# vxlerian/cpu-raymarcher

Hardware: AMD Instinct MI355X
Metric: frames/sec, 3840x2160 Dense-Grid sphere-trace (+ avg SDF-calls/pixel) (higher is better)
Workload: dtype f64

## Files before the change

### cpu_raymarcher_amd/_native.py

```python
import ctypes as C
import os
import subprocess

_PKG = os.path.dirname(os.path.abspath(__file__))
LIB_PATH = os.environ.get("RM_HIP_LIB") or os.path.join(_PKG, "librm_hip.so")
CSRC = os.path.join(_PKG, "csrc")

RM_OK = 0
RM_E_INVALID = -1
RM_E_UNSUPPORTED = -2
RM_E_NO_DEVICE = -3
RM_E_HIP = -4
RM_E_NO_SCENE = -5
RM_E_NOMEM = -6
RM_SCENE_UPLOADED = -(2 ** 31)

_STATUS_NAMES = {0: "RM_OK", -1: "RM_E_INVALID", -2: "RM_E_UNSUPPORTED", -3: "RM_E_NO_DEVICE",
                 -4: "RM_E_HIP", -5: "RM_E_NO_SCENE", -6: "RM_E_NOMEM"}


class RmError(RuntimeError):
    def __init__(self, code, msg):
        super().__init__("%s (%d): %s" % (_STATUS_NAMES.get(code, "?"), code, msg))
        self.code = code
# ... 207 lines not shown
    "rm_scene_field_device": (C.c_int, [_VP, C.POINTER(rm_lattice), _VP, _VP, _VP, _VP]),
    "rm_scene_points": (C.c_int, [_VP, C.POINTER(rm_point_query), C.c_int64, _VP, _VP, _VP, _VP, _VP, _VP, _VP]),
    "rm_scene_points_device": (C.c_int, [_VP, C.POINTER(rm_point_query), C.c_int64, _VP, _VP, _VP, _VP, _VP, _VP, _VP, _VP]),
    "rm_lattice_points": (C.c_int, [C.POINTER(rm_lattice), C.c_int64, C.c_int64, _VP]),
    "rm_shade_field_device": (C.c_int, [_VP, C.POINTER(rm_field_shade), C.c_int64, _VP, _VP, _VP]),
    "rm_shade_field": (C.c_int, [_VP, C.POINTER(rm_field_shade), C.c_int64, _VP, _VP]),
    "rm_mesh_field_device": (C.c_int, [_VP, C.POINTER(rm_lattice), _VP, C.c_int32, C.c_double, _VP, C.c_int64, _VP, C.c_int64, _VP, _VP]),
    "rm_scene_mesh": (C.c_int, [_VP, C.POINTER(rm_lattice), C.c_double, _VP, C.c_int64, _VP, C.c_int64, C.POINTER(rm_mesh_info)]),
    "rm_mesh_cells_device": (C.c_int, [_VP, C.POINTER(rm_lattice), _VP, C.c_int32, C.c_double, _VP, C.c_int64, _VP, _VP]),
    "rm_scene_sharpen_device": (C.c_int, [_VP, C.POINTER(rm_lattice), C.POINTER(rm_sharp_query), C.c_int64, _VP, _VP, _VP, _VP, _VP]),
    "rm_scene_sharpen": (C.c_int, [_VP, C.POINTER(rm_lattice), C.POINTER(rm_sharp_query), C.c_int64, _VP, _VP, _VP, _VP]),
    "rm_lattice_blocks": (C.c_int, [C.POINTER(rm_lattice), C.POINTER(C.c_int32)]),
    "rm_scene_blocks_device": (C.c_int, [_VP, C.POINTER(rm_lattice), C.c_double, C.c_double, _VP, _VP, _VP, _VP, _VP]),
    "rm_scene_tiles_device": (C.c_int, [_VP, C.POINTER(rm_lattice), _VP, C.c_int64, _VP, _VP]),
    "rm_scene_edit_balls": (C.c_int, [_VP, C.POINTER(rm_sphere_edit), C.c_int32, C.POINTER(rm_ball), C.c_int32, C.POINTER(C.c_int32)]),
    "rm_scene_tiles_update_device": (C.c_int, [_VP, C.POINTER(rm_lattice), _VP, _VP, C.c_int64, _VP, C.c_int32, _VP, C.c_int64, _VP, _VP, _VP, _VP]),
    "rm_mesh_tiles_device": (C.c_int, [_VP, C.POINTER(rm_lattice), _VP, _VP, C.c_int64, _VP, C.c_double, _VP, C.c_int64, _VP, C.c_int64, _VP, _VP,
                                       _VP, _VP]),
    "rm_scene_mesh_sparse": (C.c_int, [_VP, C.POINTER(rm_lattice), C.c_double, C.c_double, _VP, C.c_int64, _VP, C.c_int64, _VP, _VP,
                                       C.POINTER(rm_mesh_info), C.POINTER(rm_sparse_info)]),
    "rm_measure_field_device": (C.c_int, [_VP, C.POINTER(rm_lattice), _VP, C.c_int32, C.c_double, _VP, _VP]),
    "rm_measure_tiles_device": (C.c_int, [_VP, C.POINTER(rm_lattice), _VP, _VP, C.c_int64, _VP, _VP, C.c_double, _VP, _VP]),
    "rm_scene_measure": (C.c_int, [_VP, C.POINTER(rm_lattice), C.c_double, C.c_double, C.POINTER(rm_measure), C.POINTER(rm_sparse_info)]),
    "rm_measure_world": (C.c_int, [C.POINTER(rm_lattice), C.POINTER(rm_measure), C.POINTER(rm_measure_world)]),
    "rm_label_field_device": (C.c_int, [_VP, C.POINTER(rm_lattice), _VP, C.c_int32, C.c_double, C.c_int32, _VP, _VP, _VP]),
    "rm_measure_labels_device": (C.c_int, [_VP, C.POINTER(rm_lattice), _VP, C.c_int64, _VP, _VP]),
    "rm_scene_parts": (C.c_int, [_VP, C.POINTER(rm_lattice), C.c_double, C.c_int32, _VP, C.c_int64, _VP, C.POINTER(rm_parts_info)]),
    "rm_ray_march": (C.c_int, [_VP, C.POINTER(rm_ray_query), C.c_int64, _VP, _VP, _VP, _VP, _VP, _VP]),
    "rm_ray_march_device": (C.c_int, [_VP, C.POINTER(rm_ray_query), C.c_int64, _VP, _VP, _VP, _VP, _VP, _VP, _VP]),
    "rm_camera_rays": (C.c_int, [C.c_int32, C.c_int32, C.c_double, C.c_double, C.c_int32, C.c_int32, _VP, _VP]),
    "rm_ray_pick": (C.c_int, [_VP, C.POINTER(rm_ray_query), C.c_int64, _VP, _VP, _VP, _VP, _VP, _VP, _VP]),
    "rm_ray_pick_device": (C.c_int, [_VP, C.POINTER(rm_ray_query), C.c_int64, _VP, _VP, _VP, _VP, _VP, _VP, _VP, _VP]),
    "rm_ray_light": (C.c_int, [_VP, C.POINTER(rm_ray_query), C.POINTER(rm_light), C.c_int64, _VP, _VP, _VP, _VP, _VP, _VP, _VP, _VP, _VP,
                               _VP]),
    "rm_ray_light_device": (C.c_int, [_VP, C.POINTER(rm_ray_query), C.POINTER(rm_light), C.c_int64, _VP, _VP, _VP, _VP, _VP, _VP, _VP, _VP,
                                      _VP, _VP, _VP]),
    "rm_ray_walk": (C.c_int, [_VP, C.POINTER(rm_ray_query), C.c_int64, _VP, _VP, C.c_int32, _VP, _VP]),
    "rm_ray_walk_device": (C.c_int, [_VP, C.POINTER(rm_ray_query), C.c_int64, _VP, _VP, C.c_int32, _VP, _VP, _VP]),
    "rm_phong_light": (C.c_int, [_VP]),
    "rm_shade_lit_device": (C.c_int, [_VP, C.c_int32, C.c_int32, C.c_int32, _VP, _VP, _VP, _VP, _VP, _VP]),
    "rm_shade_lit": (C.c_int, [_VP, C.c_int32, C.c_int32, C.c_int32, _VP, _VP, _VP, _VP, _VP]),
    "rm_scene_object": (C.c_int, [_VP, C.c_int32, C.POINTER(rm_node), C.c_int32, C.POINTER(C.c_int32)]),
    "rm_render_tile": (C.c_int, [_VP, C.POINTER(rm_job), _VP, _VP, _VP, _VP]),
    "rm_render_tile_device": (C.c_int, [_VP, C.POINTER(rm_job), C.c_int32, _VP, _VP, _VP, _VP, _VP, _VP]),
    "rm_render_frames_device": (C.c_int, [_VP, C.POINTER(rm_job), C.c_int32, _VP, C.c_int32, _VP, _VP, _VP, _VP, _VP, _VP, _VP]),
    "rm_compare_frames_device": (C.c_int, [_VP, C.c_int32, C.c_int32, C.c_int32, C.POINTER(rm_frame_set), C.POINTER(rm_frame_set),
                                           C.c_int32, C.c_int32, _VP, _VP, _VP]),
    "rm_compare_frames": (C.c_int, [_VP, C.c_int32, C.c_int32, C.c_int32, C.POINTER(rm_frame_set), C.POINTER(rm_frame_set),
                                    C.c_int32, C.c_int32, _VP, _VP]),
    "rm_counter_hist_device": (C.c_int, [_VP, C.c_int32, C.c_int32, C.c_int32, _VP, _VP, _VP, C.c_int32, C.c_int32, C.c_int32, C.c_int32,
                                         _VP, _VP]),
    "rm_counter_hist": (C.c_int, [_VP, C.c_int32, C.c_int32, C.c_int32, _VP, _VP, _VP, C.c_int32, C.c_int32, C.c_int32, C.c_int32, _VP]),
    "rm_shade_ranged_device": (C.c_int, [_VP, C.c_int32, C.c_int32, C.c_int32, C.c_int32, _VP, _VP, C.c_uint32, C.c_uint32, _VP, _VP]),
    "rm_shade_ranged": (C.c_int, [_VP, C.c_int32, C.c_int32, C.c_int32, C.c_int32, _VP, _VP, C.c_uint32, C.c_uint32, _VP]),
    "rm_sweep_views": (C.c_int, [C.c_double, C.c_double, C.c_double, C.c_double, C.c_double, C.c_double, C.c_int32, _VP]),
    "rm_render_stripes_device": (C.c_int, [_VP, C.POINTER(rm_job), C.c_int32, C.c_int32, C.c_int32, C.c_int32,
                                           _VP, _VP, _VP, _VP, _VP, _VP]),
    "rm_stripe_rows": (C.c_int, [C.c_int32, C.c_int32, C.c_int32, C.c_int32, C.c_int32]),
    "rm_deal_stripes": (C.c_int, [C.c_int32, C.c_int32, C.c_int32, _VP, _VP]),
    "rm_render_stripe_list_device": (C.c_int, [_VP, C.POINTER(rm_job), C.c_int32, C.c_int32, _VP, C.c_int32,
                                               _VP, _VP, _VP, _VP, _VP, _VP]),
    "rm_assemble_frame_device": (C.c_int, [_VP, _VP, C.c_int64, C.c_int64, C.c_int32, C.c_int32, C.c_int32, _VP,
                                           C.c_int32, C.c_int32, _VP, C.c_int64, _VP, _VP]),
    "rm_shade": (C.c_int, [_VP, C.c_int32, C.c_int32, C.c_int32, _VP, _VP, _VP, _VP, _VP]),
    "rm_shade_device": (C.c_int, [_VP, C.c_int32, C.c_int32, C.c_int32, _VP, _VP, _VP, _VP, _VP, _VP]),
    "rm_reduce_counters": (C.c_int, [_VP, _VP, _VP, C.c_int64, C.POINTER(rm_diagnostics)]),
    "rm_reduce_counters_device": (C.c_int, [_VP, _VP, _VP, C.c_int64, C.POINTER(rm_diagnostics), _VP]),
    "rm_reduce_counters_enqueue": (C.c_int, [_VP, _VP, _VP, C.c_int64, _VP, _VP]),
    "rm_render_attach_diagnostics": (C.c_int, [_VP, _VP]),
    "rm_partition_rows": (C.c_int, [C.c_int32, C.c_int32, C.c_int32, C.POINTER(C.c_int32), C.POINTER(C.c_int32)]),
    "rm_selftest_hypot": (C.c_int, [_VP, _VP, C.c_int64, _VP]),
    "rm_selftest_fastdiv": (C.c_int, [_VP, C.c_uint64, C.c_int64, C.POINTER(C.c_uint64)]),
    "rm_selftest_recip": (C.c_int, [_VP, C.c_int, _VP]),
    "rm_debug_read_stamps": (C.c_int, [_VP, _VP]),
    "rm_debug_read_wave_times": (C.c_int, [_VP, _VP]),
    "rm_debug_read_batch_log": (C.c_int, [_VP, _VP]),
    "rm_debug_read_counts": (C.c_int, [_VP, _VP]),
    "rm_debug_read_lpt_costs": (C.c_int, [_VP, _VP, C.c_int64]),
    "rm_debug_launch_fill": (C.c_int, [_VP, C.c_int32, C.POINTER(C.c_int32)]),
    "rm_debug_last_launch": (C.c_int, [_VP, C.POINTER(C.c_uint32)]),
    "rm_debug_overlap_fill": (C.c_int, [_VP, C.c_int32, C.c_int64, C.POINTER(C.c_int32)]),
    "rm_debug_step_box": (C.c_int, [_VP, C.POINTER(C.c_int32)]),
    "rm_debug_cell_tab": (C.c_int, [_VP, C.POINTER(C.c_int32)]),
    "rm_debug_exact_tree": (C.c_int, [_VP, C.POINTER(C.c_int32)]),
    "rm_debug_rect_cull": (C.c_int, [_VP, _VP, _VP, C.c_int32, C.c_int32, C.POINTER(C.c_int32)]),
    "rm_debug_leaf_rects": (C.c_int, [_VP, _VP, _VP, C.c_int32, C.c_int32, _VP, _VP, C.c_int64, C.POINTER(C.c_int64)]),
    "rm_rtc_source": (C.c_int, [_VP, C.c_char_p, C.c_int64, C.POINTER(C.c_int64)]),
    "rm_rtc_compile_check": (C.c_int, [_VP, C.c_int32, C.c_int32, C.c_char_p, C.c_int64, C.POINTER(C.c_double)]),
    "rm_rtc_status": (C.c_int, [_VP, C.POINTER(C.c_int32), C.POINTER(C.c_int32), C.c_char_p, C.c_int64]),
    "rm_set_option": (C.c_int, [_VP, C.c_char_p, C.c_int64]),
    "rm_get_option": (C.c_int, [_VP, C.c_char_p, C.POINTER(C.c_int64)]),
}

_lib = None


def build(force=False, verbose=False):
    srcs = [os.path.join(CSRC, f) for f in os.listdir(CSRC) if f.endswith((".hip", ".cpp", ".h"))]
    srcs.append(os.path.join(os.path.dirname(_PKG), "include", "rm_raymarch.h"))
    if not force and os.path.exists(LIB_PATH) and all(
            os.path.getmtime(LIB_PATH) >= os.path.getmtime(s) for s in srcs):
        return LIB_PATH
    cmd = ["make", "-j%d" % min(8, os.cpu_count() or 1), "-C", CSRC, "all"] + (["-B"] if force else [])
    subprocess.check_call(cmd, stdout=None if verbose else subprocess.DEVNULL)
    return LIB_PATH


def lib():
    global _lib
    if _lib is None:
        if not os.path.exists(LIB_PATH):
            raise ImportError(
                "cpu_raymarcher_amd: %s is missing. Build it with `python -c 'import __graft_entry__ as g; "
                "g.build()'` or `make -C cpu_raymarcher_amd/csrc`. There is no CPU fallback." % LIB_PATH)
        try:
            import torch
        except ImportError:
            pass
        L = C.CDLL(LIB_PATH)
        for name, (res, args) in SIGNATURES.items():
            if os.environ.get("RM_HIP_LIB") and not hasattr(L, name):
                continue
            fn = getattr(L, name)
            fn.restype = res
            fn.argtypes = args
        _lib = L
    return _lib


def check(ctx, rc):
    if rc == RM_OK:
        return
    msg = lib().rm_last_error(ctx).decode() if ctx else ""
    raise (RmUnsupported if rc == RM_E_UNSUPPORTED else RmError)(rc, msg)
```

### cpu_raymarcher_amd/context.py

```python
import collections
import contextlib
import ctypes as C

import numpy as np

from . import _native as N

Points = collections.namedtuple("Points", "position dist normal object steps count")
SparseBlocks = collections.namedtuple("SparseBlocks", "slot list dist n_kept dims")
Sharp = collections.namedtuple("Sharp", "position feature count")
MeasureWorld = collections.namedtuple("MeasureWorld", "cell_volume volume centroid second projected_area area_estimate")


class Measure(collections.namedtuple("Measure", "n_points n_inside n_nonfinite sum1 sum2 crossings lo hi n_blocks n_kept n_blocks_inside")):
    world = None

    def inertia(self):
        xx, yy, zz, xy, yz, zx = self.world.second
        second = np.array([[xx, xy, zx], [xy, yy, yz], [zx, yz, zz]], np.float64)
        return np.trace(second) * np.eye(3) - second


class Parts:

# ... 128 lines not shown


def _current_stream_ptr():
    import torch
    return C.c_void_p(torch.cuda.current_stream().cuda_stream)


class Context:

    def __init__(self, device=0):
        self._h = C.c_void_p()
        self.device = -1 if device is None else int(device)
        rc = N.lib().rm_create(self.device, C.byref(self._h))
        if rc != N.RM_OK:
            raise N.RmError(rc, "rm_create(device=%d) failed: no usable HIP device" % self.device)

    def close(self):
        if self._h:
            N.lib().rm_destroy(self._h)
            self._h = C.c_void_p()

    def __del__(self):
        try:
            self.close()
        except Exception:
            pass

    def __enter__(self):
        return self

    def __exit__(self, *a):
        self.close()

    def set_option(self, key, value):
        N.check(self._h, N.lib().rm_set_option(self._h, key.encode(), int(value)))

    def get_option(self, key):
        v = C.c_int64(0)
        N.check(self._h, N.lib().rm_get_option(self._h, key.encode(), C.byref(v)))
        return v.value

    @contextlib.contextmanager
    def _exact(self, exact):
        if not exact:
            yield
            return
        before = self.get_option("exact")
        self.set_option("exact", 1)
        try:
            yield
        finally:
            self.set_option("exact", before)

    def exact_tree(self):
        out = (C.c_int32 * 4)()
        N.check(self._h, N.lib().rm_debug_exact_tree(self._h, out))
        return dict(mode=out[0], nodes=out[1], leaves=out[2], depth=out[3])

    def launch_fill(self, asked):
        v = C.c_int32(0)
        N.check(self._h, N.lib().rm_debug_launch_fill(self._h, int(asked), C.byref(v)))
        return v.value

    def last_launch(self):
        out = (C.c_uint32 * 4)()
        N.check(self._h, N.lib().rm_debug_last_launch(self._h, out))
        return dict(workgroups=out[0], threads=out[1], lds_bytes=out[2], cus=out[3])

    def overlap_fill(self, asked, items):
        v = C.c_int32(0)
        N.check(self._h, N.lib().rm_debug_overlap_fill(self._h, int(asked), int(items), C.byref(v)))
        return v.value

    def step_box(self):
        out = (C.c_int32 * 6)()
        N.check(self._h, N.lib().rm_debug_step_box(self._h, out))
        return dict(last=bool(out[0]), planned=bool(out[1]), reason=out[2], list_cap=out[3], list_cap_without=out[4], table_bytes=out[5])

    def cell_tab(self):
        out = (C.c_int32 * 12)()
        N.check(self._h, N.lib().rm_debug_cell_tab(self._h, out))
        return dict(last=bool(out[0]), planned=bool(out[1]), reason=out[2], list_cap=out[3], list_cap_without=out[4], table_bytes=out[5],
                    per_cu=out[6], scene_bytes=out[7], scene_bytes_without=out[8], cells=out[9], records=out[10], leaf_sets=out[11])

    def rect_cull(self, rot, origin, width, height):
        r = np.ascontiguousarray(rot, dtype=np.float32).reshape(9)
        o = np.ascontiguousarray(origin, dtype=np.float32).reshape(3)
        out = (C.c_int32 * 5)()
        N.check(self._h, N.lib().rm_debug_rect_cull(self._h, _ptr(r), _ptr(o), int(width), int(height), out))
        return dict(last=bool(out[0]), planned=bool(out[1]), reason=out[2], leaves=out[3], max_leaves=out[4])

    def leaf_rects(self, rot, origin, width, height):
        r = np.ascontiguousarray(rot, dtype=np.float32).reshape(9)
        o = np.ascontiguousarray(origin, dtype=np.float32).reshape(3)
        n = C.c_int64(0)
        N.check(self._h, N.lib().rm_debug_leaf_rects(self._h, _ptr(r), _ptr(o), int(width), int(height), None, None, 0, C.byref(n)))
        rects = np.zeros((max(1, n.value), 4), np.uint16)
        nodes = np.zeros(max(1, n.value), np.int32)
        N.check(self._h, N.lib().rm_debug_leaf_rects(self._h, _ptr(r), _ptr(o), int(width), int(height), _ptr(rects), _ptr(nodes),
                                                     n.value, C.byref(n)))
        return rects[:n.value], nodes[:n.value]

    def scene_from_preset(self, index, accel):
        N.check(self._h, N.lib().rm_scene_from_preset(self._h, int(index), int(accel)))

    def scene_from_spheres(self, centers, radii, accel):
        c = np.ascontiguousarray(centers, dtype=np.float32).reshape(-1, 3)
        r = np.ascontiguousarray(radii, dtype=np.float64).reshape(-1)
        if len(c) != len(r):
            raise ValueError("centers and radii differ in length")
        N.check(self._h, N.lib().rm_scene_from_spheres(self._h, _ptr(c), _ptr(r), len(r), int(accel)))

    def scene_from_prims(self, prims, accel):
        prims = list(prims)
        arr = (N.rm_prim * max(1, len(prims)))()
        for i, (t, m, par) in enumerate(prims):
            arr[i].type = int(t)
            for k in range(16):
                arr[i].world_to_local[k] = float(m[k])
            for k in range(3):
                arr[i].params[k] = float(par[k]) if k < len(par) else 0.0
        N.check(self._h, N.lib().rm_scene_from_prims(self._h, arr, len(prims), int(accel)))

    def scene_from_nodes(self, nodes, roots, accel):
        nodes = list(nodes)
        arr = (N.rm_node * max(1, len(nodes)))()
        for i, (t, a, b, m, par) in enumerate(nodes):
            arr[i].type, arr[i].child_a, arr[i].child_b = int(t), int(a), int(b)
            for k in range(16):
                arr[i].world_to_local[k] = 0.0 if m is None else float(m[k])
            for k in range(6):
                arr[i].params[k] = float(par[k]) if k < len(par) else 0.0
        r = np.ascontiguousarray(roots, dtype=np.int32)
        N.check(self._h, N.lib().rm_scene_from_nodes(self._h, arr, len(nodes), _ptr(r), len(r), int(accel)))

    def edit_spheres(self, edits):
        arr, n = self._edit_array(edits)
        N.check(self._h, N.lib().rm_scene_edit_spheres(self._h, arr, n))

    @staticmethod
    def _edit_array(edits):
        if isinstance(edits, C.Array) and edits._type_ is N.rm_sphere_edit:
            return edits, len(edits)
        edits = list(edits)
        n = len(edits)
        arr = (N.rm_sphere_edit * max(1, n))()
        for k, e in enumerate(edits):
            arr[k].op = N.EDIT_OPS[e[0]] if isinstance(e[0], str) else int(e[0])
            arr[k].index = int(e[1])
            if len(e) > 2:
                arr[k].center[:] = [float(v) for v in np.asarray(e[2], np.float32).reshape(3)]
                arr[k].radius = float(e[3])
        return arr, n

    def edit_balls(self, edits):
        arr, n = self._edit_array(edits)
        count = C.c_int32(0)
        out = np.zeros(2 * n, N.BALL_DTYPE)
        N.check(self._h, N.lib().rm_scene_edit_balls(self._h, arr, n, out.ctypes.data_as(C.POINTER(N.rm_ball)) if n else None, 2 * n, C.byref(count)))
        return out[:count.value]

    def scene_table(self, name, from_device=True):
        size = C.c_int64(0)
        key = name.encode()
        N.check(self._h, N.lib().rm_debug_scene_table(self._h, key, int(bool(from_device)), None, 0, C.byref(size)))
        out = np.zeros(size.value, np.uint8)
# ... 1126 lines not shown
```

### cpu_raymarcher_amd/csrc/rm_api.cpp

```cpp
#include <hip/hip_runtime_api.h>

#include <algorithm>
#include <array>
#include <cerrno>
#include <climits>
#include <cmath>
#include <cstdio>
#include <cstdlib>
#include <cstring>
#include <functional>
#include <limits>
#include <map>
#include <unordered_map>
#include <new>
#include <string>
#include <vector>

#include "../../include/rm_raymarch.h"
#include "rm_diag.h"
#include "rm_kernels.h"
#include "rm_rtc.h"
#include "rm_scene_host.h"

namespace {
// ... 260 lines not shown
        for (auto &u : t.users) {
            (void)hipEventSynchronize(u.second);
            (void)hipEventDestroy(u.second);
        }
        t.users.clear();
        t.valid = false;
        const size_t n = static_cast<size_t>(oct_nodes);
        if (t.nodes < n) {
            (void)hipFree(t.dev);
            t.dev = nullptr;
            t.nodes = 0;
            if (hipMalloc(reinterpret_cast<void **>(&t.dev), n * sizeof(RmOctFrameNode)) == hipSuccess) t.nodes = n;
            else (void)hipGetLastError();
        }
        if (!t.dev || rm_launch_oct_frame_table(oct, oct_nodes, origin, t.dev, stream) != hipSuccess) return nullptr;
        for (int a = 0; a < 3; ++a) t.origin[a] = origin[a];
        t.gen = gen;
        t.valid = true;
        t.builder = stream;
        if (!t.built && hipEventCreateWithFlags(&t.built, hipEventDisableTiming) != hipSuccess) t.built = nullptr;
        if (!t.built || hipEventRecord(t.built, stream) != hipSuccess) (void)hipStreamSynchronize(stream);
        cur = k;
        return &t;
    }
    static void read_by(Table &t, hipStream_t stream) {
        hipEvent_t ev = nullptr;
        for (auto &u : t.users)
            if (u.first == stream) ev = u.second;
        if (!ev) {
            if (hipEventCreateWithFlags(&ev, hipEventDisableTiming) == hipSuccess) t.users.emplace_back(stream, ev);
            else ev = nullptr;
        }
        if (ev) (void)hipEventRecord(ev, stream);
        else (void)hipStreamSynchronize(stream);
    }
    void release() {
        for (Table &t : slots) {
            (void)hipFree(t.dev);
            for (auto &u : t.users) (void)hipEventDestroy(u.second);
            if (t.built) (void)hipEventDestroy(t.built);
        }
    }
};

}

struct rm_ctx {
    int device = -1;
    bool has_device = false;
    std::string err = "";
    hipStream_t stream = nullptr;

    bool have_scene = false;
    bool scene_is_uploaded = false;
    int scene_preset = 0;
    rmh::HostScene host;
    DeviceScene dev;

    bool have_uploaded = false;
    SceneDesc uploaded;
    double time = 0.0;

    void *scratch = nullptr;
    size_t scratch_bytes = 0;
    hipEvent_t scratch_busy = nullptr;
    RmDiagDevice *d_diag = nullptr;
    float light[3] = {0, 0, 0};

    int64_t opt_tile_w = 8;
    bool tile_w_set = false;
    int64_t opt_filter = 1;
    int64_t opt_lds = 1;
    int64_t opt_kernel = 0;
    int64_t opt_list_cap = 32;
    int64_t opt_coop = 1;
    int64_t opt_grid = 1;
    int64_t opt_nn = 2;
    int64_t opt_ext = 1;
    int64_t opt_blocks_per_cu = 6;
    int64_t opt_lds_fill = 0;
    int64_t opt_min_fill = 1;
    int64_t opt_overlap_fill = 1;
    int hw_queues = 4;
    uint32_t last_v2_shape[6] = {0, 0, 0, 0, 0, 0};
    int64_t opt_item_wide = 0;
    int64_t opt_multi_step = 1;
    int64_t opt_step_box = 1;
    int64_t opt_cell_tab = 1;
    int64_t opt_lds_kb = 0;
    int64_t opt_refill = 64;
    int64_t opt_recs = 1;
    int64_t opt_static = 0;
    int64_t opt_lut = 1;
    int64_t opt_cull = 1;
    int64_t opt_rect_cull = 1;
    std::vector<uint16_t> cull_leaves;
    int64_t opt_rel = 1;
    int64_t opt_uniform = 1;
    int64_t opt_sub = 1;
    int64_t opt_hw_xcd = 1;
    int64_t opt_v1_lists = 1;
    int64_t opt_v1_block = 64;
    int64_t opt_oct_lean = 1;
    int64_t opt_lpt = 1;
    LaunchSlots slots;
    LptRing lpt;
    OctTableRing oct_tables;
    FrameRing frames;
    CompareRing compare;
    HistRing hists;
    unsigned long long scene_gen = 0;
    int64_t opt_n0_batch = 64;
    int64_t opt_length = 0;
    int64_t opt_exact = 0;
    bool exact_ready = false;
    int exact_mode = 0;
    rmh::ExactTree exact_tree;
    RmBvhNode *d_exact_nodes = nullptr;
    int32_t *d_exact_ids = nullptr;
    const char *last_kernel = "";
    std::string last_kernel_kept;
    int64_t opt_device_build = 1;
    int64_t opt_specialise = 1;
    int64_t opt_rtc_spheres = 16;
    int64_t opt_prune = 1;
    std::string rtc_src;
    std::map<int, rmrtc::Kernel> rtc_kernels;
    std::vector<rmrtc::Kernel> rtc_owned;
    std::map<int, std::string> rtc_failed;
    std::string rtc_log;
    struct V2Special {
        int launches = 0;
        int state = 0;
        bool lite = false;
        rmrtc::Kernel k;
    };
    std::unordered_map<uint64_t, V2Special> v2_special;
    int64_t opt_v2_after = 3;
    struct DevTable {
        std::vector<int32_t> host;
        int32_t *dev = nullptr;
    };
    std::vector<DevTable> tables;
    int64_t opt_item_px = 128;
    void *diag_next = nullptr;
    unsigned long long *d_stamps = nullptr;
    int num_cus = 256;
};

namespace {

int fail(rm_ctx *ctx, int code, const std::string &msg) {
    if (ctx) ctx->err = msg;
    return code;
}

int hip_fail(rm_ctx *ctx, hipError_t e, const char *what) {
    return fail(ctx, RM_E_HIP, std::string(what) + ": " + hipGetErrorString(e));
}

int read_hw_queues() {
    const char *s = std::getenv("GPU_MAX_HW_QUEUES");
    if (!s || !*s) return 4;
    char *end = nullptr;
    errno = 0;
    const long long v = std::strtoll(s, &end, 10);
    if (errno || end == s || *end != '\0' || v <= 0) return 4;
    return static_cast<int>(std::min<long long>(v, INT_MAX));
}

int launch_fill(int asked, int queues, bool min_fill) {
// ... 686 lines not shown
    std::memcpy(p.light, ctx->light, sizeof p.light);
    for (int k = 0; k < 9; ++k) p.rot_d[k] = p.rot[k];
    for (int k = 0; k < 3; ++k) {
        p.origin_d[k] = p.origin[k];
        p.light_d[k] = p.light[k];
    }
    fill_scene_view(ctx, p);
    if (!std::isfinite(job->time)) return fail(ctx, RM_E_INVALID, "non-finite time");
    ctx->time = job->time;
    p.time = job->time;
    p.tile_w = static_cast<int32_t>(ctx->opt_tile_w);
    p.nodes_in_lds = static_cast<int32_t>(ctx->opt_lds);
    p.filter = static_cast<int32_t>(ctx->opt_filter);
    p.variant = static_cast<int32_t>(ctx->opt_kernel);
    if (p.variant == 0)
        p.variant = (ctx->host.accel == RM_ACCEL_OCTREE || ctx->host.spheres.size() < 8 ||
                     (ctx->opt_specialise && !ctx->rtc_src.empty() && rmrtc::available(nullptr) &&
                      static_cast<int64_t>(ctx->host.spheres.size()) < ctx->opt_rtc_spheres))
                        ? 1
                        : 2;
    if (p.algorithm != RM_ALG_SPHERE_TRACER) p.variant = 1;
    if (ctx->host.general) p.variant = 1;
    if (p.variant == 1 && !ctx->tile_w_set) p.tile_w = 8;
    p.list_cap = static_cast<int32_t>(ctx->opt_list_cap);
    p.coop = static_cast<int32_t>(ctx->opt_coop);
    p.bvh_prim_count = static_cast<int32_t>(ctx->host.bvh_prims.size());
    p.oct_prim_count = static_cast<int32_t>(ctx->host.oct_prims.size());
    p.blocks_per_cu = static_cast<int32_t>(ctx->opt_blocks_per_cu);
    p.launch_per_cu = launch_fill(p.blocks_per_cu, ctx->hw_queues, ctx->opt_min_fill != 0);
    p.overlap_per_cu = overlap_fill(p.blocks_per_cu, ctx->hw_queues, ctx->opt_min_fill != 0, ctx->opt_overlap_fill != 0);
    p.num_cus = ctx->num_cus;
    p.refill_threshold = static_cast<int32_t>(ctx->opt_refill);
    p.hw_xcd = static_cast<int32_t>(ctx->opt_hw_xcd);
    p.item_px = static_cast<int32_t>(ctx->opt_item_px);
    p.stamps = ctx->d_stamps;
    for (int k = 0; k < 3; ++k) {
        p.pq_dim[k] = ctx->host.pq_dim[k];
        p.pq_origin[k] = ctx->host.pq_origin[k];
        p.pq_inv[k] = ctx->host.pq_inv[k];
        p.pq_cell[k] = ctx->host.pq_inv[k] > 0.f ? static_cast<float>((1.0 / static_cast<double>(ctx->host.pq_inv[k])) * 0.9999) : 0.f;
    }
    p.pq_cell_count = static_cast<int32_t>(ctx->host.pq_cells.size());
    p.pq_list_count = static_cast<int32_t>(ctx->host.pq_list.size());
    p.use_grid = (ctx->opt_grid && !ctx->host.pq_cells.empty()) ? 1 : 0;
    p.pq_cells = ctx->dev.pq_cells;
    p.pq_list = ctx->dev.pq_list;
    p.bvh_leaves = ctx->dev.bvh_leaves;
    p.bvh_leaf_count = (ctx->opt_cull && ctx->host.accel == RM_ACCEL_BVH) ? ctx->dev.bvh_leaf_count : 0;
    p.rect_cull = rect_cull_refusal(ctx, p.rot, p.origin, p.width, p.height) == 0 ? 1 : 0;
    p.nn_cells = ctx->dev.nn_cells;
    p.nn_list = ctx->dev.nn_list;
    p.nn_cell_count = static_cast<int32_t>(ctx->host.nn_cells.size());
    p.nn_list_count = static_cast<int32_t>(ctx->host.nn_list.size());
    const bool nn_on = ctx->opt_nn == 1 || (ctx->opt_nn == 2 && ctx->host.spheres.size() <= 512);
    p.use_nn = (p.use_grid && nn_on && !ctx->host.nn_cells.empty()) ? 1 : 0;
    p.leaf_order = ctx->host.leaf_order ? 1 : 0;
    p.rel_boxes = static_cast<int32_t>(ctx->opt_rel);
    p.n0_batch = static_cast<int32_t>(ctx->opt_n0_batch);
    p.v1_lists = static_cast<int32_t>(ctx->opt_v1_lists);
    p.v1_block = static_cast<int32_t>(ctx->opt_v1_block);
    p.oct_lean = static_cast<int32_t>(ctx->opt_oct_lean);
    p.v1_list_offset = -1;
    p.prim_filter = (ctx->opt_filter && ctx->host.general && !ctx->host.program && ctx->host.prim_filter_ok &&
                     ctx->host.spheres.size() == ctx->host.prims.size()) ? 1 : 0;
    p.lds_budget_kb = static_cast<int32_t>(ctx->opt_lds_kb);
    p.lds_fill = static_cast<int32_t>(ctx->opt_lds_fill);
    p.item_wide = static_cast<int32_t>(ctx->opt_item_wide);
    p.multi_step = static_cast<int32_t>(ctx->opt_multi_step);
    p.step_tab = ctx->dev.step_tab;
    p.sb_bins = ctx->host.sb_bins;
    p.sb_stride = ctx->host.sb_stride;
    for (int k = 0; k < 3; ++k) {
        p.sb_origin[k] = ctx->host.sb_origin[k];
        p.sb_inv[k] = ctx->host.sb_inv[k];
    }
    p.step_box = (ctx->opt_step_box && ctx->opt_multi_step && ctx->host.accel == RM_ACCEL_BVH && !ctx->host.step_tab.empty() &&
                  (ctx->dev.step_tab || !ctx->has_device)) ? 1 : 0;
    p.cell_tab = ctx->dev.cell_tab;
    p.ct_rec_off = ctx->host.ct_rec_off;
    p.ct_list_off = ctx->host.ct_list_off;
    p.ct_words = static_cast<int32_t>(ctx->host.cell_tab.size());
    for (int k = 0; k < 3; ++k) p.ct_dim[k] = ctx->host.ct_dim[k];
    p.cell_on = (ctx->opt_cell_tab && p.step_box && !ctx->host.cell_tab.empty() && (ctx->dev.cell_tab || !ctx->has_device)) ? 1 : 0;
    p.uniform_radius = 0;
    if (ctx->opt_uniform && !ctx->host.general && ctx->host.spheres.size() >= 2 &&
        ctx->host.spheres.size() <= 256) {
        const auto &sp = ctx->host.spheres;
        const auto &rd = ctx->host.radii;
        bool same = rd.size() == sp.size();
        for (size_t k = 1; same && k < sp.size(); ++k)
            same = std::memcmp(&sp[k].rf, &sp[0].rf, sizeof(float)) == 0 && std::memcmp(&rd[k], &rd[0], sizeof(double)) == 0;
        p.uniform_radius = same ? 1 : 0;
    }
    for (int k = 0; k < 3; ++k) {
        p.nn_dim[k] = ctx->host.nn_dim[k];
        p.nn_inv[k] = ctx->host.nn_inv[k];
    }
    p.oct_recs = ctx->opt_recs ? ctx->dev.oct_recs : nullptr;
    p.oct_sub_hdr = (ctx->opt_sub && ctx->opt_recs) ? ctx->dev.oct_sub_hdr : nullptr;
    p.oct_sub_list = ctx->dev.oct_sub_list;
    return RM_OK;
}

template <typename Launch>
int read_mismatches(rm_ctx *ctx, Launch launch, uint64_t *mismatches) {
    RM_HIP(ctx, hipSetDevice(ctx->device));
    Staging st{ctx};
    const size_t o = st.region(sizeof(unsigned long long));
    const int rc = st.reserve();
    if (rc) return rc;
    RM_HIP(ctx, st.zero(o, sizeof(unsigned long long)));
    RM_HIP(ctx, launch(st.at<unsigned long long>(o)));
    unsigned long long h = 0;
    RM_HIP(ctx, st.out(&h, o, sizeof h));
    RM_HIP(ctx, st.sync());
    *mismatches = h;
    return RM_OK;
}

int norm_shader(int s) { return (s >= RM_SHADE_NORMAL && s <= RM_SHADE_ITERATION_HEATMAP) ? s : RM_SHADE_NORMAL; }

int fill_query_params(rm_ctx *ctx, const rm_ray_query *q, RmRenderParams &p) {
    const double scene_time = ctx->time;
    rm_job job;
    std::memset(&job, 0, sizeof job);
    job.width = 1;
    job.height = 1;
    job.y_end = 1;
    job.time = q->time;
    const bool known = q->algorithm >= RM_ALG_SPHERE_TRACER && q->algorithm <= RM_ALG_ADAPTIVE_STEP_V3;
    job.algorithm = known ? q->algorithm : RM_ALG_SPHERE_TRACER;
    job.scene_preset_index = ctx->scene_is_uploaded ? RM_SCENE_UPLOADED : ctx->scene_preset;
    job.acceleration_structure = ctx->host.accel;
    job.overshoot_factor = q->overshoot_factor;
    job.step_size = q->step_size;
    const int rc = fill_params(ctx, &job, p);
    ctx->time = scene_time;
    p.rtc_function = nullptr;
    return rc;
}

int check_query(rm_ctx *ctx, const rm_ray_query *q, int64_t n, const void *origins, const void *dirs) {
    if (!q) return fail(ctx, RM_E_INVALID, "null query");
    if (n < 0 || n > std::numeric_limits<int32_t>::max()) return fail(ctx, RM_E_INVALID, "ray count out of range");
    if (n > 0 && (!origins || !dirs)) return fail(ctx, RM_E_INVALID, "null ray buffer");
    if (!ctx->has_device) return fail(ctx, RM_E_NO_DEVICE, "host-only context: there is no CPU ray path");
    if (!ctx->have_scene) return fail(ctx, RM_E_NO_SCENE, "no scene set");
    return RM_OK;
}

template <typename Args>
struct RayCall {
    RmRays rays;
    Args args;
    hipError_t (*launch[2])(const RmRenderParams &, const RmRays &, const Args &, hipStream_t, const char **);
    int64_t chunk;
    int n_cols;
    Column cols[kMaxColumns];
    void column(const void *ptr, size_t bytes, void *slot, bool in, bool out = true) { cols[n_cols++] = Column{ptr, bytes, slot, in, out}; }
};

template <typename Args, typename Check, typename Describe>
int ray_call(rm_ctx *ctx, const rm_ray_query *q, int64_t n, const void *origins, const void *dirs, bool host, void *stream, Check check,
             Describe describe) {
    if (!ctx) return RM_E_INVALID;
    int rc = check();
// ... 2405 lines not shown
    if (asked < 1 || asked > 8) return fail(ctx, RM_E_INVALID, "blocks_per_cu must be in [1, 8]");
    if (items < 0) return fail(ctx, RM_E_INVALID, "items must not be negative");
    const bool min_fill = ctx->opt_min_fill != 0;
    *effective = rm_v2_overlap_per_cu(launch_fill(asked, ctx->hw_queues, min_fill),
                                      overlap_fill(asked, ctx->hw_queues, min_fill, ctx->opt_overlap_fill != 0), items, ctx->num_cus);
    return RM_OK;
}

int rm_debug_last_launch(rm_ctx *ctx, uint32_t out[4]) {
    if (!ctx || !out) return RM_E_INVALID;
    for (int k = 0; k < 3; ++k) out[k] = ctx->last_v2_shape[k];
    out[3] = static_cast<uint32_t>(ctx->num_cus);
    return RM_OK;
}

int rm_debug_step_box(rm_ctx *ctx, int32_t out[6]) {
    if (!ctx || !out) return RM_E_INVALID;
    for (int k = 0; k < 6; ++k) out[k] = 0;
    out[0] = static_cast<int32_t>(ctx->last_v2_shape[3]);
    if (!ctx->have_scene) return fail(ctx, RM_E_NO_SCENE, "no scene set");
    rm_job job;
    std::memset(&job, 0, sizeof job);
    job.width = job.height = job.y_end = 64;
    job.algorithm = RM_ALG_SPHERE_TRACER;
    job.scene_preset_index = ctx->scene_is_uploaded ? RM_SCENE_UPLOADED : ctx->scene_preset;
    job.acceleration_structure = ctx->host.accel;
    job.overshoot_factor = job.step_size = std::nan("");
    const double scene_time = ctx->time;
    RmRenderParams p;
    const int rc = fill_params(ctx, &job, p);
    ctx->time = scene_time;
    if (rc) return rc;
    out[5] = static_cast<int32_t>(ctx->host.step_tab.size() * sizeof(uint32_t));
    RmRenderParams plain = p;
    plain.step_box = 0;
    out[4] = rm_v2_plan(plain).list_cap;
    const RmV2Plan plan = rm_v2_plan(p);
    out[3] = plan.list_cap;
    const bool v2 = p.variant == 2 && p.algorithm == 0 && p.accel == 2;
    out[1] = v2 && plan.step_box ? 1 : 0;
    out[2] = out[1] ? 0 : (ctx->host.step_tab.empty() && v2 && ctx->opt_step_box && ctx->opt_multi_step ? 2 : (v2 && plan.refused ? 3 : 1));
    return RM_OK;
}

int rm_debug_cell_tab(rm_ctx *ctx, int32_t out[12]) {
    if (!ctx || !out) return RM_E_INVALID;
    for (int k = 0; k < 12; ++k) out[k] = 0;
    out[0] = static_cast<int32_t>(ctx->last_v2_shape[5]);
    if (!ctx->have_scene) return fail(ctx, RM_E_NO_SCENE, "no scene set");
    rm_job job;
    std::memset(&job, 0, sizeof job);
    job.width = job.height = job.y_end = 64;
    job.algorithm = RM_ALG_SPHERE_TRACER;
    job.scene_preset_index = ctx->scene_is_uploaded ? RM_SCENE_UPLOADED : ctx->scene_preset;
    job.acceleration_structure = ctx->host.accel;
    job.overshoot_factor = job.step_size = std::nan("");
    const double scene_time = ctx->time;
    RmRenderParams p;
    const int rc = fill_params(ctx, &job, p);
    ctx->time = scene_time;
    if (rc) return rc;
    const auto &tab = ctx->host.cell_tab;
    out[5] = static_cast<int32_t>(tab.size() * sizeof(uint32_t));
    if (!tab.empty()) {
        out[9] = static_cast<int32_t>(tab[0] * tab[1] * tab[2]);
        out[10] = static_cast<int32_t>(tab[3]);
        out[11] = static_cast<int32_t>(tab[7]);
    }
    RmRenderParams plain = p;
    plain.cell_on = 0;
    const RmV2Plan without = rm_v2_plan(plain);
    out[4] = without.list_cap;
    out[8] = static_cast<int32_t>(without.lds ? without.scene_bytes : 0);
    const RmV2Plan plan = rm_v2_plan(p);
    out[3] = plan.list_cap;
    out[6] = plan.per_cu;
    out[7] = static_cast<int32_t>(plan.lds ? plan.scene_bytes : 0);
    const bool v2 = p.variant == 2 && p.algorithm == 0 && p.accel == 2;
    out[1] = v2 && plan.cell_on ? 1 : 0;
    out[2] = out[1] ? 0 : (tab.empty() && v2 && ctx->opt_cell_tab && ctx->opt_step_box && ctx->opt_multi_step ? 2 : (v2 && plan.cell_refused ? 3 : 1));
    return RM_OK;
}

int rm_debug_exact_tree(rm_ctx *ctx, int32_t out[4]) {
    if (!ctx || !out) return RM_E_INVALID;
    for (int k = 0; k < 4; ++k) out[k] = 0;
    if (!ctx->have_scene) return fail(ctx, RM_E_NO_SCENE, "no scene set");
    const int rc = ensure_exact_tree(ctx);
    if (rc) return rc;
    out[0] = ctx->exact_mode;
    if (ctx->exact_mode == 1) {
        out[1] = static_cast<int32_t>(ctx->host.bvh.size());
        out[2] = ctx->host.bvh_leaves;
        out[3] = ctx->host.bvh_depth;
    } else if (ctx->exact_mode == 2) {
        out[1] = static_cast<int32_t>(ctx->exact_tree.nodes.size());
        out[2] = ctx->exact_tree.leaves;
        out[3] = ctx->exact_tree.depth;
    }
    return RM_OK;
}

int rm_debug_rect_cull(rm_ctx *ctx, const float *rot9, const float *origin3, int32_t width, int32_t height, int32_t out[5]) {
    if (!ctx || !out || !rot9 || !origin3) return RM_E_INVALID;
    for (int k = 0; k < 5; ++k) out[k] = 0;
    out[0] = static_cast<int32_t>(ctx->last_v2_shape[4]);
    out[4] = RM_RECT_CULL_MAX_LEAVES;
    if (!ctx->have_scene) return fail(ctx, RM_E_NO_SCENE, "no scene set");
    rm_job job;
    std::memset(&job, 0, sizeof job);
    job.width = job.height = job.y_end = 64;
    job.algorithm = RM_ALG_SPHERE_TRACER;
    job.scene_preset_index = ctx->scene_is_uploaded ? RM_SCENE_UPLOADED : ctx->scene_preset;
    job.acceleration_structure = ctx->host.accel;
    job.overshoot_factor = job.step_size = std::nan("");
    const double scene_time = ctx->time;
    RmRenderParams p;
    const int rc = fill_params(ctx, &job, p);
    ctx->time = scene_time;
    if (rc) return rc;
    out[3] = static_cast<int32_t>(ctx->cull_leaves.size());
    const bool v2 = p.variant == 2 && p.algorithm == 0 && p.accel == 2;
    out[2] = v2 ? rect_cull_refusal(ctx, rot9, origin3, width, height) : 1;
    out[1] = out[2] == 0 ? 1 : 0;
    return RM_OK;
}

int rm_debug_leaf_rects(rm_ctx *ctx, const float *rot9, const float *origin3, int32_t width, int32_t height, uint16_t *rects,
                        int32_t *nodes, int64_t cap, int64_t *n) {
    if (!ctx || !n || !rot9 || !origin3 || cap < 0) return RM_E_INVALID;
    *n = 0;
    int32_t why[5];
    const int rc = rm_debug_rect_cull(ctx, rot9, origin3, width, height, why);
    if (rc) return rc;
    if (!why[1]) return RM_OK;
    *n = static_cast<int64_t>(ctx->cull_leaves.size());
    for (int64_t j = 0; j < *n && j < cap; ++j) {
        const RmBvhNode &nd = ctx->host.bvh[ctx->cull_leaves[static_cast<size_t>(j)]];
        const RmLeafRect r = rm_leaf_rect(nd.lo, nd.hi, origin3, rot9, width, height);
        if (rects) {
            rects[4 * j] = r.x_lo;
            rects[4 * j + 1] = r.x_hi;
            rects[4 * j + 2] = r.y_lo;
            rects[4 * j + 3] = r.y_hi;
        }
        if (nodes) nodes[j] = ctx->cull_leaves[static_cast<size_t>(j)];
    }
    return RM_OK;
}

enum OptionKind {
    kSwitch,
    kRange,
    kZeroOrRange,
    kSet,
};
struct OptionRow {
    const char *key;
    int64_t rm_ctx::*member;
    OptionKind kind;
    int64_t v[4];
    const char *error;
};
static const OptionRow kOptions[] = {
    {"tile_w", &rm_ctx::opt_tile_w, kSet, {8, 16, 32, 64}, "tile_w must be 8, 16, 32 or 64"},
    {"filter", &rm_ctx::opt_filter, kSwitch, {}, nullptr},
    {"nodes_in_lds", &rm_ctx::opt_lds, kSwitch, {}, nullptr},
    {"kernel", &rm_ctx::opt_kernel, kRange, {0, 2}, "kernel must be 0 (auto), 1 or 2"},
    {"list_cap", &rm_ctx::opt_list_cap, kRange, {1, 64}, "list_cap must be in [1, 64]"},
    {"coop", &rm_ctx::opt_coop, kSwitch, {}, nullptr},
    {"recs", &rm_ctx::opt_recs, kSwitch, {}, nullptr},
    {"lut", &rm_ctx::opt_lut, kSwitch, {}, nullptr},
    {"uniform", &rm_ctx::opt_uniform, kSwitch, {}, nullptr},
    {"lds_kb", &rm_ctx::opt_lds_kb, kZeroOrRange, {16, 64}, "lds_kb must be 0 (auto) or in [16, 64]"},
    {"multi_step", &rm_ctx::opt_multi_step, kSwitch, {}, nullptr},
    {"step_box", &rm_ctx::opt_step_box, kSwitch, {}, nullptr},
    {"cell_tab", &rm_ctx::opt_cell_tab, kSwitch, {}, nullptr},
    {"item_wide", &rm_ctx::opt_item_wide, kSwitch, {}, nullptr},
    {"prune", &rm_ctx::opt_prune, kSwitch, {}, nullptr},
    {"rtc_spheres", &rm_ctx::opt_rtc_spheres, kRange, {0, 33}, "rtc_spheres must be 0..33"},
    {"specialise_v2_after", &rm_ctx::opt_v2_after, kRange, {0, 1000000}, "specialise_v2_after must be 0 (never) .. 1000000 launches"},
    {"specialise", &rm_ctx::opt_specialise, kRange, {0, 2}, "specialise must be 0, 1 or 2"},
    {"lds_fill", &rm_ctx::opt_lds_fill, kSwitch, {}, nullptr},
    {"min_fill", &rm_ctx::opt_min_fill, kSwitch, {}, nullptr},
    {"overlap_fill", &rm_ctx::opt_overlap_fill, kSwitch, {}, nullptr},
    {"cull", &rm_ctx::opt_cull, kSwitch, {}, nullptr},
    {"rect_cull", &rm_ctx::opt_rect_cull, kSwitch, {}, nullptr},
    {"rel", &rm_ctx::opt_rel, kSwitch, {}, nullptr},
    {"static", &rm_ctx::opt_static, kRange, {0, 95}, "static must be in [0, 95] percent"},
    {"sub", &rm_ctx::opt_sub, kSwitch, {}, nullptr},
    {"refill", &rm_ctx::opt_refill, kRange, {1, 64}, "refill must be in [1, 64]"},
    {"item_px", &rm_ctx::opt_item_px, kSet, {64, 128, 256, 256}, "item_px must be 64, 128 or 256"},
    {"hw_xcd", &rm_ctx::opt_hw_xcd, kSwitch, {}, nullptr},
    {"grid", &rm_ctx::opt_grid, kSwitch, {}, nullptr},
    {"nn", &rm_ctx::opt_nn, kRange, {0, 2}, "nn must be 0 (off), 1 (on) or 2 (auto)"},
    {"ext", &rm_ctx::opt_ext, kSwitch, {}, nullptr},
    {"blocks_per_cu", &rm_ctx::opt_blocks_per_cu, kRange, {1, 8}, "blocks_per_cu must be in [1, 8]"},
    {"v1_lists", &rm_ctx::opt_v1_lists, kSwitch, {}, nullptr},
    {"v1_block", &rm_ctx::opt_v1_block, kSet, {64, 128, 256, 256}, "v1_block must be 64, 128 or 256"},
    {"oct_lean", &rm_ctx::opt_oct_lean, kSwitch, {}, nullptr},
    {"lpt", &rm_ctx::opt_lpt, kSwitch, {}, nullptr},
    {"n0_batch", &rm_ctx::opt_n0_batch, kRange, {1, 64}, "n0_batch must be in [1, 64]"},
    {"device_build", &rm_ctx::opt_device_build, kSwitch, {}, nullptr},
    {"length", &rm_ctx::opt_length, kRange, {0, 1}, "length must be 0 (Math.hypot) or 1 (Math.sqrt)"},
    {"exact", &rm_ctx::opt_exact, kRange, {0, 1}, "exact must be 0 (Scene.getDistance) or 1 (the exact field)"},
};

static const OptionRow *find_option(const char *key) {
    for (const OptionRow &o : kOptions)
        if (!std::strcmp(key, o.key)) return &o;
    return nullptr;
}

int rm_set_option(rm_ctx *ctx, const char *key, int64_t value) {
    if (!ctx || !key) return RM_E_INVALID;
    const OptionRow *o = find_option(key);
    if (!o) return fail(ctx, RM_E_INVALID, std::string("unknown option ") + key);
    bool ok = true;
    switch (o->kind) {
        case kSwitch: value = value ? 1 : 0; break;
        case kRange: ok = value >= o->v[0] && value <= o->v[1]; break;
        case kZeroOrRange: ok = value == 0 || (value >= o->v[0] && value <= o->v[1]); break;
        case kSet: ok = std::find(std::begin(o->v), std::end(o->v), value) != std::end(o->v); break;
    }
    if (!ok) return fail(ctx, RM_E_INVALID, o->error);
    const bool changed = ctx->*(o->member) != value;
    ctx->*(o->member) = value;
    if (o->member == &rm_ctx::opt_tile_w) ctx->tile_w_set = true;
    if (o->member == &rm_ctx::opt_length && changed && ctx->have_scene) {
        ctx->have_scene = false;
        return ensure_scene(ctx, ctx->scene_is_uploaded ? RM_SCENE_UPLOADED : ctx->scene_preset, ctx->host.accel);
    }
    return RM_OK;
}

int rm_get_option(const rm_ctx *ctx, const char *key, int64_t *value) {
    if (!ctx || !key || !value) return RM_E_INVALID;
    const OptionRow *o = find_option(key);
    if (!o) return RM_E_INVALID;
    *value = ctx->*(o->member);
    return RM_OK;
}

}
```

### cpu_raymarcher_amd/csrc/rm_kernels.h

```cpp
#pragma once
#ifndef __HIPCC_RTC__
#include <hip/hip_runtime_api.h>
#include <stddef.h>
#include <stdint.h>
#endif

#include "rm_types.h"

struct RmDiagDevice {
    unsigned long long total_sdf;
    unsigned long long total_iters;
    unsigned int max_sdf;
    unsigned int min_sdf;
    unsigned long long pad;
};

#ifdef RM_LENGTH_SQRT
#define RM_LEN_VARIANT(name) name##_sqrt
#define RM_LEN_TAG " [length=sqrt]"
#define RM_LEN_IS_SQRT true
#else
#define RM_LEN_VARIANT(name) name
#define RM_LEN_TAG ""
#define RM_LEN_IS_SQRT false
#endif

inline __host__ __device__ RmLeafRect rm_leaf_rect(const float lo[3], const float hi[3], const float o[3], const float rot[9], int W, int H) {
    const RmLeafRect whole = {0, 65535, 0, 65535}, none = {65535, 0, 65535, 0};
    double ql[3], qh[3];
    for (int k = 0; k < 3; ++k) {
        ql[k] = static_cast<double>(lo[k]) - static_cast<double>(o[k]);
        qh[k] = static_cast<double>(hi[k]) - static_cast<double>(o[k]);
    }
    double umin = 0.0, umax = 0.0, vmin = 0.0, vmax = 0.0;
    bool behind = false;
#pragma unroll 1
    for (int corner = 0; corner < 8; ++corner) {
        const double qx = (corner & 1) ? qh[0] : ql[0], qy = (corner & 2) ? qh[1] : ql[1], qz = (corner & 4) ? qh[2] : ql[2];
        const double z = -(qx * rot[6] + qy * rot[7] + qz * rot[8]);
        const double a = qx * rot[0] + qy * rot[1] + qz * rot[2];
        const double b = qx * rot[3] + qy * rot[4] + qz * rot[5];
        if (!(z > 1e-6 * (__builtin_fabs(qx) + __builtin_fabs(qy) + __builtin_fabs(qz)))) behind = true;
        const double u = a / z, v = b / z;
        if (corner == 0 || u < umin) umin = u;
        if (corner == 0 || u > umax) umax = u;
        if (corner == 0 || v < vmin) vmin = v;
        if (corner == 0 || v > vmax) vmax = v;
    }
    if (behind) return whole;
    const double mu = __builtin_fmax(1.0 / W, 1e-4), mv = __builtin_fmax(1.0 / H, 1e-4);
    const double xl = ((umin - mu - 1e-6 * (1.0 + __builtin_fabs(umin))) * 0.5 + 0.5) * W;
    const double xh = ((umax + mu + 1e-6 * (1.0 + __builtin_fabs(umax))) * 0.5 + 0.5) * W;
    const double yl = ((vmin - mv - 1e-6 * (1.0 + __builtin_fabs(vmin))) * 0.5 + 0.5) * H;
    const double yh = ((vmax + mv + 1e-6 * (1.0 + __builtin_fabs(vmax))) * 0.5 + 0.5) * H;
    if (!(xl - xl == 0.0 && xh - xh == 0.0 && yl - yl == 0.0 && yh - yh == 0.0)) return whole;
    if (xh < 0.0 || yh < 0.0 || xl > W - 1.0 || yl > H - 1.0) return none;
    RmLeafRect r;
    r.x_lo = static_cast<uint16_t>(xl <= 0.0 ? 0 : (xl >= 65535.0 ? 65535 : static_cast<int>(__builtin_floor(xl))));
    r.x_hi = static_cast<uint16_t>(xh >= 65535.0 ? 65535 : static_cast<int>(__builtin_ceil(xh)));
    r.y_lo = static_cast<uint16_t>(yl <= 0.0 ? 0 : (yl >= 65535.0 ? 65535 : static_cast<int>(__builtin_floor(yl))));
    r.y_hi = static_cast<uint16_t>(yh >= 65535.0 ? 65535 : static_cast<int>(__builtin_ceil(yh)));
    return r;
}

enum { RM_CMP_NONE = -1, RM_CMP_SDF = 0, RM_CMP_ITERS = 1, RM_CMP_DEPTH = 2, RM_CMP_NORMAL = 3, RM_CMP_SURFACE = 4 };
struct RmCompareStats {
    unsigned long long pixels;
    unsigned long long sums[14];
    unsigned int max_abs_depth, max_abs_normal;
};
struct RmComparePartial {
    unsigned long long v[16];
};
struct RmCompareArgs {
    const uint8_t *depth_a, *depth_b, *normal_a, *normal_b;
    const uint16_t *sdf_a, *sdf_b, *iters_a, *iters_b;
    uint8_t *rgba;
    RmCompareStats *stats;
    RmComparePartial *partials;
    unsigned int *counters;
    long long npx;
    unsigned int gain;
};

constexpr int RM_HIST_NBINS = 256;
struct RmCounterHist {
    unsigned long long pixels, sum;
    unsigned int min, max, range_lo, range_hi, shift, reserved;
    unsigned int bins[RM_HIST_NBINS];
};
struct RmFrameHist {
    RmCounterHist sdf, iters;
};
struct RmHistScratch {
    unsigned int bins[2][RM_HIST_NBINS];
    unsigned long long sum[2];
    unsigned int max[2], inv_min[2];
    unsigned int ticket, pad[3];
};
struct RmHistArgs {
    const uint16_t *sdf, *iters;
    const uint8_t *normal;
    RmFrameHist *hist;
    RmHistScratch *scratch;
    long long npx;
    unsigned int shift, lo_permille, hi_permille;
    unsigned int want_surface;
};
struct RmShadeRangedArgs {
    const uint16_t *values;
    const RmFrameHist *hist;
    uint8_t *rgba;
    long long npx;
    unsigned int counter, lo, hi;
};
struct RmShadeLitArgs {
    const uint8_t *depth, *normal;
    const float *lit, *ao;
    uint8_t *rgba;
    long long npx;
    double light[3];
};
struct RmRays {
    const float *origins, *dirs;
    long long n;
};
struct RmQueryArgs {
    int32_t want_normal, pad;
    const int32_t *slot_obj;
    double *t;
    uint32_t *iters, *sdf;
    float *normal;
    int32_t *object;
};
struct RmLightArgs {
    const float *origins, *dirs;
    double *t;
    uint32_t *iters, *sdf;
    float *normal;
    float *lit, *ao;
    uint32_t *iters2, *sdf2;
    long long n;
    double bias, ao_step, ao_strength;
    float light[3];
    int ao_samples;
};
struct RmWalkStep {
// ... 180 lines not shown
    uint32_t *totals;
    RmPartsInfo *info;
    long long n;
    unsigned int nu, nv, nw, n_blocks;
    int f32, outside;
};
struct RmPartsMeasureArgs {
    const int32_t *labels;
    RmMeasure *records;
    long long n;
    unsigned int nu, nv, nw, n_records;
};
struct RmCandGrid {
    double org[3], w[3];
    int32_t dim[3];
    int32_t first, n, pad;
};
#define RM_CAND_NO_LIST 0xFFFFFFFFu
struct RmCandArgs {
    const RmCandGrid *grids;
    const double *spheres;
    const int32_t *ids;
    uint32_t *counts;
    double *u;
    const uint32_t *offsets;
    long long n_cells;
    unsigned long long list_len;
    double u0;
    double root_lo[3], root_hi[3];
    int32_t n_grids, cells_per_grid, n_spheres, n_ids, use_root, pad;
};
struct RmEmptyDistArgs {
    const float *boxes, *prim_lo, *prim_hi;
    double *out;
    int32_t n_nodes, n_prims;
};

#ifndef __HIPCC_RTC__
static_assert(sizeof(RmLattice) == 96, "the lattice's four vectors");
static_assert(sizeof(RmFieldArgs) == 152 && offsetof(RmFieldArgs, dist) == 96, "RmFieldArgs layout");
static_assert(sizeof(RmSharpArgs) == 176 && offsetof(RmSharpArgs, iso) == 96, "RmSharpArgs layout");
static_assert(sizeof(RmMeshArgs) == 200 && offsetof(RmMeshArgs, values) == 96, "RmMeshArgs layout");
static_assert(sizeof(RmBlocksArgs) == 184 && offsetof(RmBlocksArgs, iso) == 96, "RmBlocksArgs layout");
static_assert(sizeof(RmTilesArgs) == 168 && offsetof(RmTilesArgs, list) == 96, "RmTilesArgs layout");
static_assert(sizeof(RmSparseMeshArgs) == 232 && offsetof(RmSparseMeshArgs, iso) == 96, "RmSparseMeshArgs layout");

hipError_t rm_launch_cand_count(const RmCandArgs &a, hipStream_t stream);
hipError_t rm_launch_cand_fill(const RmCandArgs &a, void *list, int elem_bytes, hipStream_t stream);
hipError_t rm_launch_empty_dist(const RmEmptyDistArgs &a, hipStream_t stream);
hipError_t rm_launch_hypot64(const double *xyz, int64_t n, double *out, hipStream_t stream);

hipError_t rm_launch_render(const RmRenderParams &p, hipStream_t stream, const char **kernel_name, uint32_t *v2_shape = nullptr);
hipError_t rm_launch_render_sqrt(const RmRenderParams &p, hipStream_t stream, const char **kernel_name, uint32_t *v2_shape = nullptr);

const void *rm_rtc_v2_hook(const RmRenderParams &p, int accel, bool lds, bool ur, bool rel, bool length_sqrt);

hipError_t rm_launch_render_v2(const RmRenderParams &p, hipStream_t stream, const char **kernel_name, uint32_t *shape = nullptr);
hipError_t rm_launch_render_v2_sqrt(const RmRenderParams &p, hipStream_t stream, const char **kernel_name, uint32_t *shape = nullptr);

#define RM_V2_OVERLAP_ITEMS_PER_WAVE 3
inline int rm_v2_overlap_per_cu(int floor_per_cu, int candidate, long long items, int cus) {
    if (candidate <= floor_per_cu || cus <= 0) return floor_per_cu;
    const long long needed = (items + 3) / 4, resident = static_cast<long long>(cus) * candidate;
    const long long waves = 4 * (needed < resident ? needed : resident);
    return items >= RM_V2_OVERLAP_ITEMS_PER_WAVE * waves ? candidate : floor_per_cu;
}

inline bool rm_rect_cull_camera_ok(const float rot[9], const float origin[3]) {
    for (int k = 0; k < 3; ++k)
        if (!(origin[k] - origin[k] == 0.f)) return false;
    for (int i = 0; i < 3; ++i)
        for (int j = i; j < 3; ++j) {
            double d = 0.0;
            for (int k = 0; k < 3; ++k) d += static_cast<double>(rot[3 * i + k]) * static_cast<double>(rot[3 * j + k]);
            const double err = d - (i == j ? 1.0 : 0.0);
            if (!(err >= -1e-6 && err <= 1e-6)) return false;
        }
    return true;
}

struct RmV2Plan {
    bool lds, rel;
    int list_cap, step_box, tier, refused, cell_on, cell_refused;
    int per_cu;
    size_t scene_bytes, list_bytes;
};
RmV2Plan rm_v2_plan(const RmRenderParams &p);

hipError_t rm_launch_wave_distance(const RmRenderParams &p, const float *points, int64_t n, double *dist, uint32_t *count, hipStream_t stream);
hipError_t rm_launch_wave_distance_sqrt(const RmRenderParams &p, const float *points, int64_t n, double *dist, uint32_t *count, hipStream_t stream);

hipError_t rm_launch_oct_frame_table(const RmOctNode *nodes, int n, const double origin[3], RmOctFrameNode *out, hipStream_t stream);

hipError_t rm_launch_shade(int shader, int64_t n, const uint8_t *depth, const uint8_t *normal,
                           const uint16_t *sdf, const uint16_t *iters, uint8_t *rgba,
                           const float light[3], hipStream_t stream);

hipError_t rm_launch_reduce_init(RmDiagDevice *acc, hipStream_t stream);

hipError_t rm_launch_reduce(const uint16_t *sdf, const uint16_t *iters, int64_t n, RmDiagDevice *acc,
                            hipStream_t stream);

hipError_t rm_launch_distance(const RmRenderParams &p, const float *points, int64_t n, double *dist,
                              uint32_t *count, hipStream_t stream);
hipError_t rm_launch_distance_sqrt(const RmRenderParams &p, const float *points, int64_t n, double *dist,
                                   uint32_t *count, hipStream_t stream);

hipError_t rm_launch_cast(const RmRenderParams &p, const RmRays &r, const RmQueryArgs &a, hipStream_t stream, const char **kernel_name);
hipError_t rm_launch_cast_sqrt(const RmRenderParams &p, const RmRays &r, const RmQueryArgs &a, hipStream_t stream, const char **kernel_name);
hipError_t rm_launch_pick(const RmRenderParams &p, const RmRays &r, const RmQueryArgs &a, hipStream_t stream, const char **kernel_name);
hipError_t rm_launch_pick_sqrt(const RmRenderParams &p, const RmRays &r, const RmQueryArgs &a, hipStream_t stream, const char **kernel_name);
hipError_t rm_launch_light(const RmRenderParams &p, const RmRays &r, const RmLightArgs &a, hipStream_t stream, const char **kernel_name);
hipError_t rm_launch_light_sqrt(const RmRenderParams &p, const RmRays &r, const RmLightArgs &a, hipStream_t stream, const char **kernel_name);
hipError_t rm_launch_walk(const RmRenderParams &p, const RmRays &r, const RmWalkArgs &a, hipStream_t stream, const char **kernel_name);
hipError_t rm_launch_walk_sqrt(const RmRenderParams &p, const RmRays &r, const RmWalkArgs &a, hipStream_t stream, const char **kernel_name);

hipError_t rm_launch_field(const RmRenderParams &p, const RmFieldArgs &a, hipStream_t stream, const char **kernel_name);
hipError_t rm_launch_field_sqrt(const RmRenderParams &p, const RmFieldArgs &a, hipStream_t stream, const char **kernel_name);

hipError_t rm_launch_points(const RmRenderParams &p, const RmPointArgs &a, hipStream_t stream, const char **kernel_name);
hipError_t rm_launch_points_sqrt(const RmRenderParams &p, const RmPointArgs &a, hipStream_t stream, const char **kernel_name);

hipError_t rm_launch_sharp(const RmRenderParams &p, const RmSharpArgs &a, hipStream_t stream, const char **kernel_name);
hipError_t rm_launch_sharp_sqrt(const RmRenderParams &p, const RmSharpArgs &a, hipStream_t stream, const char **kernel_name);

hipError_t rm_launch_mesh(const RmMeshArgs &a, hipStream_t stream, const char **kernel_name);
hipError_t rm_launch_mesh_cells(const RmMeshArgs &a, long long *cells, hipStream_t stream, const char **kernel_name);

hipError_t rm_launch_blocks(const RmRenderParams &p, const RmBlocksArgs &a, hipStream_t stream, const char **kernel_name);
hipError_t rm_launch_blocks_sqrt(const RmRenderParams &p, const RmBlocksArgs &a, hipStream_t stream, const char **kernel_name);
hipError_t rm_launch_blocks_compact(const RmBlocksArgs &a, hipStream_t stream);
hipError_t rm_launch_tiles(const RmRenderParams &p, const RmTilesArgs &a, hipStream_t stream, const char **kernel_name);
hipError_t rm_launch_tiles_sqrt(const RmRenderParams &p, const RmTilesArgs &a, hipStream_t stream, const char **kernel_name);
hipError_t rm_launch_mesh_tiles(const RmSparseMeshArgs &a, hipStream_t stream, const char **kernel_name);
hipError_t rm_launch_tiles_update(const RmRenderParams &p, const RmTilesArgs &a, const RmTilesUpdateArgs &u, hipStream_t stream, const char **kernel_name);
hipError_t rm_launch_tiles_update_sqrt(const RmRenderParams &p, const RmTilesArgs &a, const RmTilesUpdateArgs &u, hipStream_t stream, const char **kernel_name);
hipError_t rm_launch_tiles_update_totals(const int32_t *reused, unsigned int n_kept, RmTilesUpdateInfo *info, hipStream_t stream);
unsigned int rm_measure_field_groups(long long n, unsigned int nv, unsigned int nw, int num_cus);
unsigned int rm_measure_block_groups(unsigned int n_blocks, int num_cus);
hipError_t rm_launch_measure_field(const RmMeasureFieldArgs &a, unsigned int n_groups, hipStream_t stream, const char **kernel_name);
hipError_t rm_launch_measure_tiles(const RmMeasureTilesArgs &a, unsigned int n_groups, hipStream_t stream, const char **kernel_name);
hipError_t rm_launch_label_field(const RmPartsArgs &a, hipStream_t stream, const char **kernel_name);
hipError_t rm_launch_measure_labels(const RmPartsMeasureArgs &a, int num_cus, hipStream_t stream, const char **kernel_name);

hipError_t rm_launch_frames(const RmRenderParams &p, const RmFrameView *views, int32_t n_views, RmFrameDiagBlock *blocks, RmDiagDevice *acc,
                            hipStream_t stream, const char **kernel_name);
hipError_t rm_launch_frames_sqrt(const RmRenderParams &p, const RmFrameView *views, int32_t n_views, RmFrameDiagBlock *blocks, RmDiagDevice *acc,
                                 hipStream_t stream, const char **kernel_name);

hipError_t rm_launch_lpt_sort(const uint8_t *cost_prev, uint16_t *perm, int stride, int tiles_x, int tiles_y, hipStream_t stream);

hipError_t rm_launch_assemble(const unsigned char *gathered, int64_t rank_stride, int64_t section_offset, int32_t row_bytes,
                              int32_t height, int32_t stripe_rows, const int32_t *stripe_src, int32_t n_stripes,
                              unsigned char *frame, int64_t acc_offset, int32_t world, RmDiagDevice *acc, hipStream_t stream);

int32_t rm_compare_blocks_per_frame(int64_t npx, int32_t n_frames);
hipError_t rm_launch_compare(const RmCompareArgs &a, int32_t map, int32_t n_frames, int32_t blocks_per_frame, hipStream_t stream,
                             const char **kernel_name);

hipError_t rm_launch_hist(const RmHistArgs &a, bool masked, int32_t n_frames, int32_t blocks_per_frame, hipStream_t stream,
                          const char **kernel_name);
hipError_t rm_launch_shade_ranged(const RmShadeRangedArgs &a, int32_t n_frames, hipStream_t stream, const char **kernel_name);
hipError_t rm_launch_shade_lit(const RmShadeLitArgs &a, int32_t n_frames, hipStream_t stream, const char **kernel_name);
hipError_t rm_launch_shade_field(const RmShadeFieldArgs &a, hipStream_t stream, const char **kernel_name);

hipError_t rm_launch_hypot(const float *xyz, int64_t n, double *out, hipStream_t stream);
// ... 6 lines not shown
```

### cpu_raymarcher_amd/csrc/rm_render_v2.hip

```cpp
#ifndef __HIPCC_RTC__
#include <hip/hip_runtime.h>
#endif

#include "rm_device.h"
#ifdef RM_RTC_V2
#include "rm_v2_fixed.inc"
#endif

#ifdef RM_COUNTS
__shared__ unsigned int rm_cnt_s[32];
#define RM_CNT(i)                                                                                  \
    {                                                                                              \
        const unsigned int n_ = static_cast<unsigned int>(__popcll(__ballot(1)));                  \
        const int l_ = static_cast<int>(__lane_id());                                              \
        if (__builtin_amdgcn_readfirstlane(l_) == l_) {                                            \
            atomicAdd(&rm_cnt_s[i], 1u);                                                           \
            atomicAdd(&rm_cnt_s[(i) + 16], n_);                                                    \
        }                                                                                          \
    }
__shared__ unsigned int rm_cnt_e[8];
#define RM_CNT_END(i)                                                                              \
    {                                                                                              \
        const unsigned int n_ = static_cast<unsigned int>(__popcll(__ballot(1)));                  \
        const int l_ = static_cast<int>(__lane_id());                                              \
        if (__builtin_amdgcn_readfirstlane(l_) == l_) {                                            \
            atomicAdd(&rm_cnt_e[i], 1u);                                                           \
            atomicAdd(&rm_cnt_e[(i) + 4], n_);                                                     \
        }                                                                                          \
    }
#else
#define RM_CNT(i) {}
#define RM_CNT_END(i) {}
#endif

#include "rm_bvh_list.h"
#include "rm_kernels.h"
#include "rm_diag.h"

namespace {

using namespace rmd;

#ifdef RM_STAMPS
#define RM_T0() unsigned long long t_prev_ = __builtin_amdgcn_s_memtime(); unsigned long long t_acc_[8] = {0, 0, 0, 0, 0, 0, 0, 0}; \
    const unsigned long long t_start_ = __builtin_amdgcn_s_memrealtime();                                                          \
    if (lane == 0 && P.stamps) atomicMin(&P.stamps[6], t_start_);                                                                  \
    if (lane == 0 && P.stamps && blockIdx.x * 4 + (threadIdx.x >> 6) < 8192) P.stamps[40 + blockIdx.x * 4 + (threadIdx.x >> 6)] = t_start_;
#define RM_T(i)                                                  \
    {                                                            \
        const unsigned long long t_now_ = __builtin_amdgcn_s_memtime(); \
        t_acc_[i] += t_now_ - t_prev_;                           \
        t_prev_ = t_now_;                                        \
    }
#define RM_TEND()                                                                      \
    if (lane == 0 && P.stamps) {                                                        \
        for (int i_ = 0; i_ < 8; ++i_) if (i_ != 6) atomicAdd(&P.stamps[i_], t_acc_[i_]); \
        const unsigned long long first_ = atomicMin(&P.stamps[6], t_start_);            \
        const unsigned long long rel_ = __builtin_amdgcn_s_memrealtime() - (first_ < t_start_ ? first_ : t_start_); \
        unsigned long long b_ = rel_ / 6400ull;                    \
        atomicAdd(&P.stamps[8 + (b_ > 31 ? 31 : b_)], 1ull);                            \
        if (blockIdx.x * 4 + (threadIdx.x >> 6) < 8192) P.stamps[40 + 8192 + blockIdx.x * 4 + (threadIdx.x >> 6)] = __builtin_amdgcn_s_memrealtime(); \
    }
#else
#define RM_T0()
#define RM_T(i)
#define RM_TEND()
#endif

enum Phase : int { PH_MARCH = 0, PH_N0 = 1, PH_N1 = 2, PH_N2 = 3, PH_N3 = 4, PH_DONE = 5 };

struct WaveDiag {
    unsigned long long sdf[8], iters[8];
    unsigned int mx[8], mn_inv[8];
};
__device__ __forceinline__ void wave_diag_add(WaveDiag *w, int lane, uint32_t count, uint32_t iters) {
    const unsigned int c16 = count & 0xFFFFu, i16 = iters & 0xFFFFu;
    const int k = lane & 7;
    atomicAdd(&w->sdf[k], static_cast<unsigned long long>(c16));
    atomicAdd(&w->iters[k], static_cast<unsigned long long>(i16));
    atomicMax(&w->mx[k], c16);
    atomicMax(&w->mn_inv[k], 0xFFFFFFFFu - c16);
}

__device__ __forceinline__ float wave_min_f32(float v) {
    int b = __float_as_int(v);
#define RM_DPP_MIN(ctrl, rowmask)                                                              \
    {                                                                                          \
        const float o = __int_as_float(__builtin_amdgcn_update_dpp(b, b, ctrl, rowmask, 0xF, false)); \
        const float c = __int_as_float(b);                                                     \
        b = __float_as_int(o < c ? o : c);                                                     \
    }
    RM_DPP_MIN(0xB1, 0xF)
    RM_DPP_MIN(0x4E, 0xF)
    RM_DPP_MIN(0x141, 0xF)
    RM_DPP_MIN(0x140, 0xF)
    RM_DPP_MIN(0x142, 0xA)
    RM_DPP_MIN(0x143, 0xC)
#undef RM_DPP_MIN
    return __int_as_float(__builtin_amdgcn_readlane(b, 63));
}

__device__ __forceinline__ double masked_min_f64(double v, unsigned long long mask, double init) {
    const int lo = __double2loint(v), hi = __double2hiint(v);
// ... 107 lines not shown
                                    uint32_t &count, int lane, bool coop, bool filter, bool use_grid,
                                    unsigned long long *dbg_fallback_cycles) {
    double closest = RM_MAX_DIST;
    uint32_t found = 0;
    bool walk_tree = false;
    bool in_root = false;
    if (need && use_grid) {
        const RmBvhNode root = S.nodes[0];
        if (box_contains(root.lo, root.hi, q)) {
            const int cx = min(max(static_cast<int>((q.x - P.pq_origin[0]) * P.pq_inv[0]), 0), P.pq_dim[0] - 1);
            const int cy = min(max(static_cast<int>((q.y - P.pq_origin[1]) * P.pq_inv[1]), 0), P.pq_dim[1] - 1);
            const int cz = min(max(static_cast<int>((q.z - P.pq_origin[2]) * P.pq_inv[2]), 0), P.pq_dim[2] - 1);
            in_root = true;
            const uint32_t cell = P.pq_cells[(cz * P.pq_dim[1] + cy) * P.pq_dim[0] + cx];
            const int ccnt = static_cast<int>(cell & 0xFFu);
            if (ccnt == 255) walk_tree = true;
            else {
                const uint16_t *lst = P.pq_list + (cell >> 8);
                for (int e = 0; e < ccnt; ++e) {
                    const RmBvhNode node = S.nodes[lst[e]];
                    if (!box_contains(node.lo, node.hi, q)) continue;
                    const int first = node.leaf >> 8, cnt = node.leaf & 0xFF;
                    const int32_t *ids = P.leaf_order ? nullptr : S.bvh_prims + first;
                    closest = (filter && cnt >= 2) ? lane_min_filtered(S, ids, cnt, q, closest, first)
                                                   : lane_min_exact(S, ids, cnt, q, closest, first);
                    found += static_cast<uint32_t>(cnt);
                }
            }
        }
    }
    if (need && (!use_grid || walk_tree)) {
        int i = 0;
        const int n = S.bvh_nodes;
        while (i < n) {
            const RmBvhNode node = S.nodes[i];
            if (!box_contains(node.lo, node.hi, q)) {
                i = node.skip;
                continue;
            }
            if (node.leaf < 0) {
                i = i + 1;
                continue;
            }
            const int first = node.leaf >> 8, cnt = node.leaf & 0xFF;
            const int32_t *ids = P.leaf_order ? nullptr : S.bvh_prims + first;
            closest = (filter && cnt >= 2) ? lane_min_filtered(S, ids, cnt, q, closest, first)
                                           : lane_min_exact(S, ids, cnt, q, closest, first);
            found += static_cast<uint32_t>(cnt);
            i = node.skip;
        }
    }
    bool fallback = need && found == 0;
    bool served = false;
    if (fallback && P.use_nn && in_root) {
        const int nx = min(max(static_cast<int>((q.x - P.pq_origin[0]) * P.nn_inv[0]), 0), P.nn_dim[0] - 1);
        const int ny = min(max(static_cast<int>((q.y - P.pq_origin[1]) * P.nn_inv[1]), 0), P.nn_dim[1] - 1);
        const int nz = min(max(static_cast<int>((q.z - P.pq_origin[2]) * P.nn_inv[2]), 0), P.nn_dim[2] - 1);
        const uint32_t cell = S.nn_cells[(nz * P.nn_dim[1] + ny) * P.nn_dim[0] + nx];
        const int ccnt = static_cast<int>(cell & 0xFFu);
        if (ccnt != 255) {
            closest = prims_min_best<uint16_t>(S.spheres, S.radii, S.nn_list + (cell >> 8), ccnt, 0, q, RM_MAX_DIST);
            served = true;
        }
    }
#ifdef RM_STAMPS
    const unsigned long long t_fb0 = __builtin_amdgcn_s_memtime();
#endif
    const double all = all_prims_wave(S, fallback && !served, q, lane, coop, filter);
#ifdef RM_STAMPS
    if (dbg_fallback_cycles) *dbg_fallback_cycles += __builtin_amdgcn_s_memtime() - t_fb0;
#endif
    if (fallback) {
        if (!served) closest = all;
        count += static_cast<uint32_t>(S.n_prims);
    } else if (need) {
        count += found;
    }
    return closest;
}

struct BestScan {
    int k1;
    float hi1, lb1, lb2;
    uint32_t kbest, ksecond;
};
template <bool UR>
__device__ __forceinline__ void scan_sphere(BestScan &b, const RmSphere &s, int id, const Vec3f &p) {
    if (UR) {
        const float dx = p.x - s.cx, dy = p.y - s.cy, dz = p.z - s.cz;
        const float s2 = dx * dx + dy * dy + dz * dz;
        const uint32_t key = (__float_as_uint(s2) & 0xFFFFFF00u) | static_cast<uint32_t>(id);
        const uint32_t lo = min(key, b.kbest), hi = max(key, b.kbest);
        b.kbest = lo;
        b.ksecond = min(hi, b.ksecond);
        return;
    }
    float err;
    const float a = sphere_sdf_estimate(s, p, err);
    const float lb = a - err, hi = a + err;
    const bool better = hi < b.hi1;
    b.lb2 = __builtin_fminf(b.lb2, better ? b.lb1 : lb);
    b.k1 = better ? id : b.k1;
    b.lb1 = better ? lb : b.lb1;
    b.hi1 = better ? hi : b.hi1;
}
__device__ __forceinline__ void scan_finish_uniform(BestScan &b, float rf) {
    const float len = __builtin_amdgcn_sqrtf(b.lb2);
    const float lb = (len - rf) - (len + __builtin_fabsf(rf) + 1.0f) * 4e-6f;
    b.lb2 = b.lb2 < __builtin_inff() ? lb : __builtin_inff();
}

struct NormalAux {
    int k1;
    float lb2;
    uint32_t found;
    float rho;
    float rho_cell;
    bool ok;
};
#define RM_NRM_DELTA 0.010003f
__device__ __forceinline__ float box_margin(const float lo[3], const float hi[3], const Vec3f &p) {
    const float a = __builtin_fminf(__builtin_fminf(p.x - lo[0], p.y - lo[1]), p.z - lo[2]);
    const float b = __builtin_fminf(__builtin_fminf(hi[0] - p.x, hi[1] - p.y), hi[2] - p.z);
    return __builtin_fminf(a, b);
}

struct CellTabView {
    const uint32_t *tab;
    const uint32_t *step;
    bool on;
};
__device__ __forceinline__ int cell_axis_index(const RmRenderParams &P, const uint32_t *step, int k, float x) {
    const uint32_t *axis = step + k * P.sb_stride;
    const int last = P.ct_dim[k] - 1;
    const int b = min(max(static_cast<int>((x - P.sb_origin[k]) * P.sb_inv[k]), 0), P.sb_bins - 1);
    int i = min(static_cast<int>(reinterpret_cast<const uint8_t *>(axis)[b]), last);
    const float *T = reinterpret_cast<const float *>(axis + (P.sb_bins >> 2));
    while (i < last && T[i + 1] <= x) i += 1;
    return i;
}

template <bool UR>
__device__ double bvh_distance_wave(const RmRenderParams &P, const SceneView &S, bool need, const Vec3f &q,
                                    uint32_t &count, int lane, bool coop, bool filter, bool use_grid,
                                    unsigned long long *dbg_fallback_cycles, NormalAux *aux, const CellTabView CT) {
    aux->ok = false;
    aux->rho = 0.f;
    aux->rho_cell = 0.f;
    if (!filter) return bvh_distance_wave_seq(P, S, need, q, count, lane, coop, filter, use_grid, dbg_fallback_cycles);
    double closest = RM_MAX_DIST;
    uint32_t found = 0;
    bool walk_tree = false;
    bool in_root = false;
    float rho = __builtin_inff();
    float rho_cell = 0.f;
    uint32_t nleaf16 = 0xFFFF0000u;
    BestScan bs;
    bs.k1 = -1;
    bs.hi1 = bs.lb1 = bs.lb2 = __builtin_inff();
    bs.kbest = bs.ksecond = 0xFFFFFFFFu;
    auto scan_leaf = [&](const RmBvhNode &node) {
        const int first = node.leaf >> 8, cnt = node.leaf & 0xFF;
        for (int k = 0; k < cnt; ++k) {
            const int id = P.leaf_order ? first + k : S.bvh_prims[first + k];
            RM_CNT(8)
            scan_sphere<UR>(bs, S.spheres[id], id, q);
        }
        found += static_cast<uint32_t>(cnt);
    };
    if (CT.on) {
        if (need) {
            const int ix = cell_axis_index(P, CT.step, 0, q.x), iy = cell_axis_index(P, CT.step, 1, q.y), iz = cell_axis_index(P, CT.step, 2, q.z);
            const uint32_t r = reinterpret_cast<const uint16_t *>(CT.tab + 8)[(iz * P.ct_dim[1] + iy) * P.ct_dim[0] + ix];
            const uint32_t *rec = CT.tab + P.ct_rec_off + 3u * r;
            const uint32_t w0 = rec[0], w1 = rec[1], w2 = rec[2];
            in_root = (w0 >> 24) != 0u;
            const int cnt = static_cast<int>(w1 >> 24);
            const uint16_t *lst = reinterpret_cast<const uint16_t *>(CT.tab + P.ct_list_off) + (w2 & 0xFFFFu);
            for (int e = 0; e < cnt; ++e) {
                const int id = lst[e];
                RM_CNT(8)
                scan_sphere<UR>(bs, S.spheres[id], id, q);
            }
            found = w2 >> 16;
            nleaf16 = r << 16;
            rho = 0.f;
        }
    } else if (need && use_grid) {
        const RmBvhNode root = S.nodes[0];
        const float m_root = box_margin(root.lo, root.hi, q);
        if (m_root >= 0.f) {
            const float gx = (q.x - P.pq_origin[0]) * P.pq_inv[0], gy = (q.y - P.pq_origin[1]) * P.pq_inv[1], gz = (q.z - P.pq_origin[2]) * P.pq_inv[2];
            const int cx = min(max(static_cast<int>(gx), 0), P.pq_dim[0] - 1);
            const int cy = min(max(static_cast<int>(gy), 0), P.pq_dim[1] - 1);
            const int cz = min(max(static_cast<int>(gz), 0), P.pq_dim[2] - 1);
            in_root = true;
            {
                const float fx = gx - static_cast<float>(cx), fy = gy - static_cast<float>(cy), fz = gz - static_cast<float>(cz);
                const float in_cell = __builtin_fminf(__builtin_fminf(__builtin_fminf(fx, 1.0f - fx) * P.pq_cell[0], __builtin_fminf(fy, 1.0f - fy) * P.pq_cell[1]),
                                                      __builtin_fminf(fz, 1.0f - fz) * P.pq_cell[2]);
                rho_cell = 0.0100f + __builtin_fmaxf(in_cell, 0.f);
            }
            rho = __builtin_fmaxf(__builtin_fmaxf(__builtin_fabsf(q.x), __builtin_fabsf(q.y)), __builtin_fabsf(q.z)) < 16.0f ? m_root : 0.f;
            const uint32_t cell = S.pq_cells[(cz * P.pq_dim[1] + cy) * P.pq_dim[0] + cx];
            const int ccnt = static_cast<int>(cell & 0xFFu);
            if (ccnt == 255) walk_tree = true;
            else {
                const uint16_t *lst = S.pq_list + (cell >> 8);
                for (int e = 0; e < ccnt; ++e) {
                    RM_CNT(7)
                    const RmBvhNode node = S.nodes[lst[e]];
                    const float m = box_margin(node.lo, node.hi, q);
                    rho = __builtin_fminf(rho, __builtin_fabsf(m));
                    if (m >= 0.f) {
                        scan_leaf(node);
                        found += 0x10000u;
                    }
                }
                nleaf16 = found & 0xFFFF0000u;
                found &= 0xFFFFu;
            }
        }
    }
    if (need && !CT.on && (!use_grid || walk_tree)) {
        rho = 0.f;
        int i = 0;
        const int n = S.bvh_nodes;
        while (i < n) {
            const RmBvhNode node = S.nodes[i];
            if (!box_contains(node.lo, node.hi, q)) {
                i = node.skip;
                continue;
            }
            if (node.leaf < 0) {
                i = i + 1;
                continue;
            }
            scan_leaf(node);
            i = node.skip;
        }
    }
    const bool fallback = need && found == 0;
    bool served = false;
    if (fallback && P.use_nn && in_root) {
        const int nx = min(max(static_cast<int>((q.x - P.pq_origin[0]) * P.nn_inv[0]), 0), P.nn_dim[0] - 1);
        const int ny = min(max(static_cast<int>((q.y - P.pq_origin[1]) * P.nn_inv[1]), 0), P.nn_dim[1] - 1);
        const int nz = min(max(static_cast<int>((q.z - P.pq_origin[2]) * P.nn_inv[2]), 0), P.nn_dim[2] - 1);
        const uint32_t cell = S.nn_cells[(nz * P.nn_dim[1] + ny) * P.nn_dim[0] + nx];
        const int ccnt = static_cast<int>(cell & 0xFFu);
        if (ccnt != 255) {
            const uint16_t *lst = S.nn_list + (cell >> 8);
            for (int e = 0; e < ccnt; ++e) {
                const int id = lst[e];
                RM_CNT(9)
                scan_sphere<UR>(bs, S.spheres[id], id, q);
            }
            served = true;
        }
    }
    if (fallback && !served && P.use_ext) {
        const float gx = (q.x - P.ext_origin[0]) * P.ext_inv[0], gy = (q.y - P.ext_origin[1]) * P.ext_inv[1], gz = (q.z - P.ext_origin[2]) * P.ext_inv[2];
        const float lo = __builtin_fminf(__builtin_fminf(gx, gy), gz);
        const bool inside = lo >= 0.f && gx < static_cast<float>(P.ext_dim[0]) && gy < static_cast<float>(P.ext_dim[1]) && gz < static_cast<float>(P.ext_dim[2]);
        if (inside) {
            const uint32_t cell = S.ext_cells[(static_cast<int>(gz) * P.ext_dim[1] + static_cast<int>(gy)) * P.ext_dim[0] + static_cast<int>(gx)];
            const int ccnt = static_cast<int>(cell & 0xFFu);
            if (ccnt != 255) {
                const uint16_t *lst = S.ext_list + (cell >> 8);
                for (int e = 0; e < ccnt; ++e) {
                    const int id = lst[e];
                    RM_CNT(9)
                    scan_sphere<UR>(bs, S.spheres[id], id, q);
                }
                served = true;
            }
        }
    }
    if (fallback && !served) RM_CNT(13)
    {
        const unsigned long long unserved = __ballot(fallback && !served);
        if (unserved) {
            const int n = S.n_prims, m = __popcll(unserved);
            const bool one_by_one = coop && n > 8 && static_cast<long long>(m) * (28 * ((n + 63) / 64) + 250) < 14ll * n + 200;
            if (!one_by_one && (!UR || n <= 256)) {
                if (fallback && !served) {
                    for (int id = 0; id < n; ++id) scan_sphere<UR>(bs, S.spheres[id], id, q);
                    served = true;
                }
            }
        }
    }
    bool redo = false;
    if (UR && bs.kbest != 0xFFFFFFFFu) {
        bs.k1 = static_cast<int>(bs.kbest & 0xFFu);
        bs.lb2 = bs.ksecond == 0xFFFFFFFFu ? __builtin_inff() : __uint_as_float(bs.ksecond & 0xFFFFFF00u);
    }
    if (bs.k1 >= 0) {
        RM_CNT(10)
        const RmSphere s1 = S.spheres[bs.k1];
        if (UR) scan_finish_uniform(bs, s1.rf);
        closest = sphere_sdf_fast(s1, S.radii[bs.k1], q);
        if (closest > RM_MAX_DIST) closest = RM_MAX_DIST;
        redo = bs.lb2 <= f32_upper_bound(closest);
    }
    {
        aux->k1 = bs.k1;
        aux->lb2 = bs.lb2;
        aux->found = (found & 0xFFFFu) | nleaf16;
        aux->rho = rho;
        aux->rho_cell = rho_cell;
        aux->ok = need && in_root && found > 0 && bs.k1 >= 0 && !redo;
    }
    if (__any(redo)) {
        if (redo) RM_CNT(11)
        uint32_t dummy = 0;
        const double r = bvh_distance_wave_seq(P, S, redo, q, dummy, lane, coop, filter, use_grid, nullptr);
        if (redo) closest = r;
    }
#ifdef RM_STAMPS
    const unsigned long long t_fb0 = __builtin_amdgcn_s_memtime();
#endif
    const double all = all_prims_wave(S, fallback && !served, q, lane, coop, filter);
#ifdef RM_STAMPS
    if (dbg_fallback_cycles) *dbg_fallback_cycles += __builtin_amdgcn_s_memtime() - t_fb0;
#endif
    if (fallback) {
        if (!served) closest = all;
        count += static_cast<uint32_t>(S.n_prims);
    } else if (need) {
        count += found;
    }
    return closest;
}

__device__ __forceinline__ int oct_find(const SceneView &S, const Vec3f &p) {
    const RmOctNode *nodes = S.oct;
    if (!box_contains(nodes[0].lo, nodes[0].hi, p)) return -1;
    int i = 0;
    for (;;) {
        const int first = nodes[i].first_child;
        if (first < 0) return i;
        const float cx = nodes[i].center[0], cy = nodes[i].center[1], cz = nodes[i].center[2];
        i = first + (p.x > cx ? 1 : 0) + (p.y > cy ? 2 : 0) + (p.z > cz ? 4 : 0);
    }
}

__device__ double oct_distance_lane(const SceneView &S, int node, const Vec3f &q, uint32_t &count, bool filter) {
    if (node < 0) {
        count += static_cast<uint32_t>(S.n_prims);
        return (filter && S.n_prims >= 2) ? lane_min_filtered(S, nullptr, S.n_prims, q, RM_MAX_DIST)
                                         : lane_min_exact(S, nullptr, S.n_prims, q, RM_MAX_DIST);
    }
    const RmOctNode nd = S.oct[node];
    double closest = RM_MAX_DIST;
    if (nd.prim_count > 0) {
        const int32_t *ids = S.oct_prims + nd.prim_first;
        closest = (filter && nd.prim_count >= 2) ? lane_min_filtered(S, ids, nd.prim_count, q, closest)
                                                : lane_min_exact(S, ids, nd.prim_count, q, closest);
        count += static_cast<uint32_t>(nd.prim_count);
    } else if (nd.is_empty) {
        closest = min_dist(nd.min_distance * 0.99, closest);
    }
    return closest;
}

struct Bundle {
    float n[4][3];
};
__device__ __forceinline__ Bundle make_bundle(const RmRenderParams &C, int x0, int x1, int y0, int y1) {
    const float mu = __builtin_fmaxf(1.0f / static_cast<float>(C.width), 1e-4f);
    const float mv = __builtin_fmaxf(1.0f / static_cast<float>(C.height), 1e-4f);
    const float u0 = (static_cast<float>(x0) / static_cast<float>(C.width) - 0.5f) * 2.0f - mu;
    const float u1 = (static_cast<float>(x1) / static_cast<float>(C.width) - 0.5f) * 2.0f + mu;
    const float v0 = (static_cast<float>(y0) / static_cast<float>(C.height) - 0.5f) * 2.0f - mv;
    const float v1 = (static_cast<float>(y1) / static_cast<float>(C.height) - 0.5f) * 2.0f + mv;
    Bundle b;
#pragma unroll
    for (int k = 0; k < 3; ++k) {
        b.n[0][k] = C.rot[k] + u0 * C.rot[6 + k];
        b.n[1][k] = C.rot[k] + u1 * C.rot[6 + k];
        b.n[2][k] = C.rot[3 + k] + v0 * C.rot[6 + k];
        b.n[3][k] = C.rot[3 + k] + v1 * C.rot[6 + k];
    }
    return b;
}
__device__ __forceinline__ bool bundle_misses_box(const Bundle &b, const float lo[3], const float hi[3], const float o[3]) {
    const float ql[3] = {lo[0] - o[0], lo[1] - o[1], lo[2] - o[2]};
    const float qh[3] = {hi[0] - o[0], hi[1] - o[1], hi[2] - o[2]};
    bool miss = false;
// ... 341 lines not shown
        return l;
    };
    auto list_column = [&](const RmRenderParams &C) {
        const uint32_t end = C.lds_off[9];
        return reinterpret_cast<uint16_t *>(smem + end) + (static_cast<uint32_t>(wave) * static_cast<uint32_t>(C.list_cap)) * 64u + static_cast<uint32_t>(lane_now());
    };
    const int item_px = P.item_px;
    int home = (P.hw_xcd ? (__builtin_amdgcn_s_getreg(20 | (3 << 11)) & 7) : (static_cast<int>(blockIdx.x) & 7)) * RM_SUBQ +
               static_cast<int>((blockIdx.x >> 3) % RM_SUBQ);
    const int refill_at = P.refill_threshold;

    int tile_col = -1, tile_row = 0, qpos = item_px;
    bool no_more = false;
    unsigned int item_t0 = 0;

    enum : int { ST_PHASE = 7, ST_TRIP_SHIFT = 3, ST_TRIP_MASK = 127 << 3, ST_HAVECUR = 1 << 10, ST_PAR_SHIFT = 11, ST_PAR_MASK = 7 << 11,
                 ST_PIXEL = 1 << 14,
                 ST_LIVE_SHIFT = 15, ST_POS_SHIFT = 22, ST_OVF = 1 << 29, ST_LIST_MASK = (0x3FFF << 15) | (1 << 29) };
    Vec3f rd = {0.f, 0.f, -1.f};
    double inv0 = 0.0, inv1 = 0.0, inv2 = 0.0;
    double t = RM_MAX_DIST;
    double sA = 0.0, sB = 0.0;
    int sC = -1;
    uint32_t counters = 0;
    uint32_t pidx = 0;
    int st = PH_DONE;

    auto ray_of = [&](const RmRenderParams &C) {
        Ray r;
        r.d = rd;
        r.o = {C.origin[0], C.origin[1], C.origin[2]};
        r.od[0] = C.origin_d[0];
        r.od[1] = C.origin_d[1];
        r.od[2] = C.origin_d[2];
        return r;
    };
    auto inv_of = [&]() {
        RayInv ri;
        ri.inv[0] = inv0;
        ri.inv[1] = inv1;
        ri.inv[2] = inv2;
        ri.par[0] = (st & (1 << ST_PAR_SHIFT)) != 0;
        ri.par[1] = (st & (2 << ST_PAR_SHIFT)) != 0;
        ri.par[2] = (st & (4 << ST_PAR_SHIFT)) != 0;
        ri.any_par = (st & ST_PAR_MASK) != 0;
        return ri;
    };
    auto list_of = [&](const RmRenderParams &C) {
        RayList L;
        L.col = list_column(C);
        L.cap = list_cap;
        L.live = (st >> ST_LIVE_SHIFT) & 127;
        L.cur_pos = (st >> ST_POS_SHIFT) & 127;
        L.cnt = (st & ST_OVF) ? list_cap + 1 : L.live;
        return L;
    };
    auto keep_list = [&](const RayList &L) {
        st = (st & ~ST_LIST_MASK) | ((L.live & 127) << ST_LIVE_SHIFT) | ((L.cur_pos & 127) << ST_POS_SHIFT) | (L.cnt > list_cap ? ST_OVF : 0);
    };
    auto set_phase = [&](int ph) { st = (st & ~ST_PHASE) | ph; };
    auto nrm_x = [&]() { return __int_as_float(__double2loint(sB)); };
    auto nrm_y = [&]() { return __int_as_float(__double2hiint(sB)); };
    auto set_normal = [&](float nx, float ny, float nz) {
        sB = __hiloint2double(__float_as_int(ny), __float_as_int(nx));
        sC = __float_as_int(nz);
    };
    auto finish_march = [&](double dist_total) {
        t = dist_total;
        set_phase((t >= RM_MAX_DIST) ? PH_DONE : PH_N0);
    };
    auto store_mine = [&](const RmRenderParams &C) {
        const bool miss = t >= RM_MAX_DIST;
        const float nx = miss ? 0.f : nrm_x(), ny = miss ? 0.f : nrm_y(), nz = miss ? 0.f : __int_as_float(sC);
        store_pixel(C, static_cast<size_t>(pidx), t, nx, ny, nz, counters >> 16, counters & 0xFFFFu);
        if (C.diag_out) wave_diag_add(&wave_diag[wave], lane_now(), counters >> 16, counters & 0xFFFFu);
    };

    RM_T0()
#ifdef RM_STAMPS_LOG
    int refill_k_ = 0;
#endif
#ifdef RM_COUNTS
    if (threadIdx.x < 32) rm_cnt_s[threadIdx.x] = 0;
    if (threadIdx.x < 8) rm_cnt_e[threadIdx.x] = 0;
    __syncthreads();
#endif
    for (;;) {
        RM_T(7)
        RM_CNT(0)
        const unsigned long long idle = __ballot((st & ST_PHASE) == PH_DONE);
        const int n_idle = __popcll(idle);
        if (n_idle >= refill_at || n_idle == 64) {
            RM_CNT(1)
#ifdef RM_STAMPS_LOG
            if (lane == 0 && P.stamps && blockIdx.x * 4 + wave < 2048 && refill_k_ < 96)
                reinterpret_cast<unsigned int *>(P.stamps + 40 + 3 * 8192)[(blockIdx.x * 4 + wave) * 96 + refill_k_] =
                    static_cast<unsigned int>(__builtin_amdgcn_s_memrealtime());
            refill_k_ += 1;
#endif
            const RmRenderParams C = cold_params();
            TileQueue Q;
            Q.counters = C.tile_counters;
            Q.tile_w = C.tile_w;
            Q.item_px = C.item_px;
            Q.tile_h = 1 << C.tile_h_log2;
            Q.tiles_x = C.tiles_x;
            Q.tiles_y = C.tiles_y;
            Q.tiles_x_magic = C.tiles_x_magic;
            Q.perm = C.lpt_perm;
            Q.perm_stride = C.lpt_stride;
            const bool want_tile = !no_more && qpos >= Q.item_px;
            const int lane_r = lane_now();
            const bool rect_batch = ACCEL == 2 && C.rect_cull && n_idle == 64;
            RmLeafRect rect0 = {65535, 0, 65535, 0};
            if (rect_batch && lane_r < C.bvh_leaf_count) rect0 = C.leaf_rects[lane_r];
            if (want_tile) {
                if (C.lpt_cost_out && tile_col >= 0) {
                    const unsigned int took = (static_cast<unsigned int>(__builtin_amdgcn_s_memrealtime()) - item_t0) >> 10;
                    if (lane_r == 0) C.lpt_cost_out[static_cast<size_t>(home) * C.lpt_stride + queue_slot_of(Q, home, tile_col, tile_row)] =
                        static_cast<uint8_t>(took < 255u ? (took ? took : 1u) : 255u);
                }
#ifdef RM_STAMPS_CLAIM
                const unsigned long long tc0 = __builtin_amdgcn_s_memrealtime();
#endif
                unsigned int claim = 0;
                if (lane_r == 0) claim = atomicAdd(&Q.counters[home * RM_QSTRIDE], 1u);
                if (pull_tile(Q, home, tile_col, tile_row, lane_r, claim)) {
                    qpos = 0;
                    if (C.lpt_cost_out) item_t0 = static_cast<unsigned int>(__builtin_amdgcn_s_memrealtime());
                } else no_more = true;
#ifdef RM_STAMPS_CLAIM
                const unsigned long long tc1 = __builtin_amdgcn_s_memrealtime();
                if (lane_r == 0 && P.stamps) {
                    atomicAdd(&P.stamps[38], tc1 - tc0);
                    atomicAdd(&P.stamps[39], 1ull);
                }
#endif
            }
            const bool rect_cull_now = rect_batch && !no_more && (qpos & 63) == 0;
            unsigned long long cand0 = 0;
            bool cand_beyond = false;
            if (rect_cull_now) {
                const int bsub = qpos >> 6;
                const int bx0 = (tile_col << C.item_w_log2) + bsub * C.sub_dx, br0 = (tile_row << C.tile_h_log2) + bsub * C.sub_dy;
                const int bx1 = bx0 + C.tile_w - 1, by0 = row_to_y(C, br0), by1 = row_to_y(C, br0 + (64 >> C.tile_w_log2) - 1);
                cand0 = __ballot(rect_overlaps(rect0, bx0, bx1, by0, by1));
                for (int j0 = 64; j0 < C.bvh_leaf_count && !cand_beyond; j0 += 64)
                    cand_beyond = __any(j0 + lane_r < C.bvh_leaf_count && rect_overlaps(C.leaf_rects[j0 + lane_r], bx0, bx1, by0, by1));
            }
            const bool no_cand = rect_cull_now && cand0 == 0 && !cand_beyond;
            if ((st & (ST_PHASE | ST_PIXEL)) == (PH_DONE | ST_PIXEL)) {
                store_mine(C);
                st &= ~ST_PIXEL;
            }
            if (!no_more) {
                const int remaining = Q.item_px - qpos;
                const int rank = __builtin_amdgcn_mbcnt_hi(static_cast<unsigned int>(idle >> 32),
                                                           __builtin_amdgcn_mbcnt_lo(static_cast<unsigned int>(idle), 0u));
                const bool take = (st & ST_PHASE) == PH_DONE && rank < remaining;
                bool in_frame = false;
                const bool whole_batch = ACCEL == 2 && C.bvh_leaf_count > 0 && n_idle == 64 && (qpos & 63) == 0;
                const int batch_sub = qpos >> 6;
                Ray ray = ray_of(C);
                RayInv ri = inv_of();
                if (take) {
                    const int n = qpos + rank;
                    const int sub = n >> 6, l = n & 63;
// ... 90 lines not shown
                        else if (t > sB) {
                            RayList L = list_of(CA);
                            Interval cur;
                            cur.tEnter = sA;
                            cur.tExit = sB;
                            cur.ord = sC;
                            const bool hc = bvh_next<REL>(S, ray, inv_of(), L, sA, sC, cur);
                            keep_list(L);
                            if (!hc) {
                                st &= ~ST_HAVECUR;
                                terminate = true;
                            } else {
                                sA = cur.tEnter;
                                sB = cur.tExit;
                                sC = cur.ord;
                                if (sA > t) skip = sA - t;
                            }
                        }
                    }
                    if (terminate) {
                        finish_march(RM_MAX_DIST);
                        break;
                    }
                    if (skip > 0.0) {
                        t += skip;
                        if (t > RM_MAX_DIST) {
                            finish_march(t);
                            break;
                        }
                        continue;
                    }
                } else if (ACCEL == 1) {
                    onode = oct_find(S, p);
                    if (onode >= 0) {
                        const double skip = oct_skip(S.oct[onode], ray, t);
                        if (skip > 0.0) {
                            t += skip;
                            if (t > RM_MAX_DIST) {
                                finish_march(t);
                                break;
                            }
                            continue;
                        }
                    }
                }
                q = p;
                need = true;
                break;
            }
        }
        bool n0_go = true;
        if (ACCEL == 2) n0_go = !__any(need) || __popcll(__ballot((st & ST_PHASE) == PH_N0)) >= CA.n0_batch;
        {
            const int ph = st & ST_PHASE;
            if (ph >= PH_N0 && ph <= PH_N3 && (ph != PH_N0 || n0_go)) {
                RM_CNT(14)
                q = point_at(ray, t);
                if (ph == PH_N1) q.x = to_f32(static_cast<double>(q.x) - 0.01);
                if (ph == PH_N2) q.y = to_f32(static_cast<double>(q.y) - 0.01);
                if (ph == PH_N3) q.z = to_f32(static_cast<double>(q.z) - 0.01);
                if (ACCEL == 1) onode = oct_find(S, q);
                need = true;
            }
        }
        RM_T(1)
        if (!__any(need)) continue;

        if (need) RM_CNT(6)
        const RmRenderParams CB = cold_params();
        const SceneView SB = scene_view<ACCEL, LDS, REL>(CB, smem);
        const bool coop = CB.coop != 0, filter = CB.filter != 0;
        const bool use_grid = ACCEL == 2 && CB.use_grid != 0;
        double dist;
        const int lane_b = lane_now();
        uint32_t evaluated = 0;
        NormalAux aux;
        aux.ok = false;
        aux.k1 = 0;
        aux.lb2 = 0.f;
        aux.found = 0;
        aux.rho = 0.f;
        aux.rho_cell = 0.f;
        const bool cell_on = ACCEL == 2 && CB.cell_on != 0;
        if (ACCEL == 2) {
            CellTabView CT;
            CT.tab = LDS ? reinterpret_cast<const uint32_t *>(smem + CB.lds_off[11]) : CB.cell_tab;
            CT.step = LDS ? reinterpret_cast<const uint32_t *>(smem + CB.lds_off[10]) : CB.step_tab;
            CT.on = cell_on;
#ifdef RM_STAMPS
            unsigned long long fbc = 0;
            dist = bvh_distance_wave<UR>(CB, SB, need, q, evaluated, lane_b, coop, filter, use_grid, &fbc, &aux, CT);
            t_acc_[4] += fbc;
            t_prev_ += fbc;
#else
            dist = bvh_distance_wave<UR>(CB, SB, need, q, evaluated, lane_b, coop, filter, use_grid, nullptr, &aux, CT);
#endif
        }
        else if (ACCEL == 1) dist = need ? oct_distance_lane(SB, onode, q, evaluated, filter) : RM_MAX_DIST;
        else {
            dist = all_prims_wave(SB, need, q, lane_b, coop, filter);
            if (need) evaluated = static_cast<uint32_t>(SB.n_prims);
        }
        counters += evaluated << 16;

        RM_T(2)
        const bool fuse = ACCEL == 2 && need && (st & ST_PHASE) == PH_N0 && aux.ok && (cell_on || aux.rho > RM_NRM_DELTA);
        const bool was_marching = need && (st & ST_PHASE) == PH_MARCH;
        if (need) {
            const int ph = st & ST_PHASE;
            if (ph == PH_MARCH) {
                t += dist;
                counters += 1;
                if (dist < RM_EPSILON || t > RM_MAX_DIST) finish_march(t);
            } else if (ph == PH_N0) {
                sA = dist;
                set_phase(PH_N1);
            } else if (ph == PH_N1) {
                sB = __hiloint2double(__double2hiint(sB), __float_as_int(to_f32(sA - dist)));
                set_phase(PH_N2);
            } else if (ph == PH_N2) {
                sB = __hiloint2double(__float_as_int(to_f32(sA - dist)), __double2loint(sB));
                set_phase(PH_N3);
            } else {
                float nx = nrm_x(), ny = nrm_y(), nz = to_f32(sA - dist);
                normalize3(nx, ny, nz);
                set_normal(nx, ny, nz);
                set_phase(PH_DONE);
            }
        }
        if (ACCEL == 2 && CB.multi_step) {
            const bool go = was_marching && aux.ok && (aux.found >> 16) != 0xFFFFu && (st & ST_PHASE) == PH_MARCH;
            if (__any(go)) {
                if (go) {
                    const RmRenderParams CM = cold_params();
                    const SceneView SM = scene_view<ACCEL, LDS, REL>(CM, smem);
                    const RmSphere s1 = SM.spheres[aux.k1];
                    const double r1 = SM.radii[aux.k1];
                    const bool step_box = CM.step_box != 0;
                    float b_lo[3], b_hi[3];
                    if (step_box && CM.cell_on) {
                        const uint32_t *tab = LDS ? reinterpret_cast<const uint32_t *>(smem + CM.lds_off[10]) : CM.step_tab;
                        const uint32_t *rec = (LDS ? reinterpret_cast<const uint32_t *>(smem + CM.lds_off[11]) : CM.cell_tab) + CM.ct_rec_off + 3u * (aux.found >> 16);
                        const uint32_t w0 = rec[0], w1 = rec[1];
#pragma unroll
                        for (int k = 0; k < 3; ++k) {
                            const float *T = reinterpret_cast<const float *>(tab + k * CM.sb_stride + (CM.sb_bins >> 2));
                            b_lo[k] = T[(w0 >> (8 * k)) & 0xFFu];
                            b_hi[k] = T[(w1 >> (8 * k)) & 0xFFu];
                        }
                    } else if (step_box) {
                        const uint32_t *tab = LDS ? reinterpret_cast<const uint32_t *>(smem + CM.lds_off[10]) : CM.step_tab;
                        const int last = CM.sb_stride - (CM.sb_bins >> 2) - 2;
                        const float qk[3] = {q.x, q.y, q.z};
#pragma unroll
                        for (int k = 0; k < 3; ++k) {
                            const uint32_t *axis = tab + k * CM.sb_stride;
                            const int b = min(max(static_cast<int>((qk[k] - CM.sb_origin[k]) * CM.sb_inv[k]), 0), CM.sb_bins - 1);
                            int i = static_cast<int>(reinterpret_cast<const uint8_t *>(axis)[b]);
                            i = min(i, last);
                            const float *T = reinterpret_cast<const float *>(axis + (CM.sb_bins >> 2));
                            float lo = T[i], hi = T[i + 1];
                            while (hi <= qk[k] && i < last) {
                                i += 1;
                                lo = hi;
                                hi = T[i + 1];
                            }
                            b_lo[k] = lo;
                            b_hi[k] = hi;
                        }
                    }
                    for (;;) {
                        if ((st & ST_TRIP_MASK) >= (RM_MAX_STEPS << ST_TRIP_SHIFT)) {
                            finish_march(t);
                            break;
                        }
                        if (t < sA || t > sB) {
                            RM_CNT_END(2)
                            break;
                        }
                        const Vec3f p2 = point_at(ray, t);
                        if (step_box) {
                            if (!(p2.x >= b_lo[0] && p2.x < b_hi[0] && p2.y >= b_lo[1] && p2.y < b_hi[1] && p2.z >= b_lo[2] && p2.z < b_hi[2])) {
                                RM_CNT_END(0)
                                break;
                            }
                        } else {
                            const RmBvhNode root = SM.nodes[0];
                            bool same = box_margin(root.lo, root.hi, p2) >= 0.f;
                            uint32_t cell = 255u;
                            if (same) {
                                const float gx = (p2.x - CM.pq_origin[0]) * CM.pq_inv[0], gy = (p2.y - CM.pq_origin[1]) * CM.pq_inv[1], gz = (p2.z - CM.pq_origin[2]) * CM.pq_inv[2];
                                const int cx = min(max(static_cast<int>(gx), 0), CM.pq_dim[0] - 1);
                                const int cy = min(max(static_cast<int>(gy), 0), CM.pq_dim[1] - 1);
                                const int cz = min(max(static_cast<int>(gz), 0), CM.pq_dim[2] - 1);
                                cell = SM.pq_cells[(cz * CM.pq_dim[1] + cy) * CM.pq_dim[0] + cx];
                            }
                            const int ccnt = static_cast<int>(cell & 0xFFu);
                            if (ccnt == 255) {
                                RM_CNT_END(1)
                                break;
                            }
                            const uint16_t *lst = SM.pq_list + (cell >> 8);
                            uint32_t left = aux.found >> 16;
                            for (int k = 0; k < ccnt; ++k) {
                                const RmBvhNode node = SM.nodes[lst[k]];
                                if (box_margin(node.lo, node.hi, p2) >= 0.f) {
                                    same = same && box_margin(node.lo, node.hi, q) >= 0.f;
                                    left -= 1u;
                                }
                            }
                            if (!same || left != 0u) {
                                RM_CNT_END(0)
                                break;
                            }
                        }
                        const float ex = p2.x - q.x, ey = p2.y - q.y, ez = p2.z - q.z;
                        const float dd = __builtin_amdgcn_sqrtf(ex * ex + ey * ey + ez * ez) * 1.00001f + 1e-7f;
                        const double e = sphere_sdf_fast(s1, r1, p2);
                        if (!(aux.lb2 - dd > f32_upper_bound(e))) {
                            RM_CNT_END(3)
                            break;
                        }
                        RM_CNT(15)
                        st += 1 << ST_TRIP_SHIFT;
                        counters += (aux.found << 16) + 1u;
                        const double d2 = __builtin_fmin(e, RM_MAX_DIST);
                        t += d2;
                        if (d2 < RM_EPSILON || t > RM_MAX_DIST) {
                            finish_march(t);
                            break;
                        }
                    }
                }
            }
        }
        if (ACCEL == 2 && __any(fuse)) {
            bool stable = true;
            if (fuse && cell_on) {
                const RmRenderParams CN = cold_params();
                const uint32_t *tab = LDS ? reinterpret_cast<const uint32_t *>(smem + CN.lds_off[10]) : CN.step_tab;
                const uint32_t *rec = (LDS ? reinterpret_cast<const uint32_t *>(smem + CN.lds_off[11]) : CN.cell_tab) + CN.ct_rec_off + 3u * (aux.found >> 16);
                const uint32_t w0 = rec[0], w1 = rec[1];
                const float qk[3] = {q.x, q.y, q.z};
                float rho = __builtin_fmaxf(__builtin_fmaxf(__builtin_fabsf(q.x), __builtin_fabsf(q.y)), __builtin_fabsf(q.z)) < 16.0f ? __builtin_inff() : 0.f;
#pragma unroll
                for (int k = 0; k < 3; ++k) {
                    const float *T = reinterpret_cast<const float *>(tab + k * CN.sb_stride + (CN.sb_bins >> 2));
                    rho = __builtin_fminf(rho, __builtin_fminf(qk[k] - T[(w0 >> (8 * k)) & 0xFFu], T[(w1 >> (8 * k)) & 0xFFu] - qk[k]));
                }
                stable = rho > RM_NRM_DELTA;
            }
            if (fuse && stable) {
                const SceneView SN = scene_view<ACCEL, LDS, REL>(cold_params(), smem);
                const RmSphere s1 = SN.spheres[aux.k1];
                const double r1 = SN.radii[aux.k1];
                Vec3f qx = q, qy = q, qz = q;
                qx.x = to_f32(static_cast<double>(q.x) - 0.01);
                qy.y = to_f32(static_cast<double>(q.y) - 0.01);
                qz.z = to_f32(static_cast<double>(q.z) - 0.01);
                const double e1 = sphere_sdf_fast(s1, r1, qx), e2 = sphere_sdf_fast(s1, r1, qy), e3 = sphere_sdf_fast(s1, r1, qz);
                const double emax = __builtin_fmax(__builtin_fmax(e1, e2), e3);
                if (aux.lb2 - RM_NRM_DELTA > f32_upper_bound(emax)) {
                    counters += (3u * aux.found) << 16;
                    float nx = to_f32(sA - __builtin_fmin(e1, RM_MAX_DIST));
                    float ny = to_f32(sA - __builtin_fmin(e2, RM_MAX_DIST));
                    float nz = to_f32(sA - __builtin_fmin(e3, RM_MAX_DIST));
                    normalize3(nx, ny, nz);
                    set_normal(nx, ny, nz);
                    set_phase(PH_DONE);
                }
            }
        }
        RM_T(3)
    }
    RM_TEND()
    {
        const RmRenderParams C = cold_params();
        if (C.diag_block) {
            const WaveDiag *w = &wave_diag[wave];
            unsigned long long ts = 0, ti = 0;
            unsigned int mx = 0, mi = 0;
#pragma unroll
            for (int k = 0; k < 8; ++k) {
                ts += w->sdf[k];
                ti += w->iters[k];
                mx = w->mx[k] > mx ? w->mx[k] : mx;
                mi = w->mn_inv[k] > mi ? w->mn_inv[k] : mi;
            }
            diag_flush_wave(C.diag_block, C.diag_out, C.tile_counters, ts, ti, mx, mi, blockIdx.x * 4u + static_cast<unsigned int>(wave),
                            gridDim.x * 4u, lane_now());
        }
    }
#ifdef RM_COUNTS
    __syncthreads();
    if (threadIdx.x < 32 && P.stamps) atomicAdd(&P.stamps[8 + threadIdx.x], static_cast<unsigned long long>(rm_cnt_s[threadIdx.x]));
    if (threadIdx.x < 8 && P.stamps) atomicAdd(&P.stamps[40 + threadIdx.x], static_cast<unsigned long long>(rm_cnt_e[threadIdx.x]));
#endif
}

#ifdef RM_RTC_V2
}
extern "C" __global__ __launch_bounds__(256, RM_V2_WAVES) void rm_rtc_render_v2(const RmRenderParams P) {
    render_v2_body<RM_RTC_V2_ACCEL, RM_RTC_V2_LDS != 0, RM_RTC_V2_UR != 0, RM_RTC_V2_REL != 0>(P);
}
#else
template <int ACCEL, bool LDS, bool UR = false, bool REL = false>
__global__ __launch_bounds__(256, RM_V2_WAVES) void render_kernel_v2(const RmRenderParams P) {
    render_v2_body<ACCEL, LDS, UR, REL>(P);
}

template <bool UR>
__global__ __launch_bounds__(256) void wave_distance_kernel(const RmRenderParams P, const float *pts, int64_t n, double *dist, uint32_t *count) {
    const int64_t i = static_cast<int64_t>(blockIdx.x) * 256 + threadIdx.x;
    const bool need = i < n;
    Vec3f q;
    q.x = need ? pts[3 * i] : 0.f;
    q.y = need ? pts[3 * i + 1] : 0.f;
    q.z = need ? pts[3 * i + 2] : 0.f;
    const SceneView S = scene_view<2, false, false>(P, nullptr);
    uint32_t c = 0;
    NormalAux aux;
    const CellTabView CT = {P.cell_tab, P.step_tab, P.cell_on != 0};
    const double d = bvh_distance_wave<UR>(P, S, need, q, c, static_cast<int>(threadIdx.x & 63), P.coop != 0, P.filter != 0, P.use_grid != 0, nullptr, &aux, CT);
    if (need) {
        dist[i] = d;
        count[i] = c;
    }
}

size_t scene_lds_bytes(const RmRenderParams &p) {
    auto up = [](size_t v) { return (v + 15) & ~static_cast<size_t>(15); };
    size_t b = 0;
    if (p.accel == 2) {
        b += up(static_cast<size_t>(p.bvh_nodes) * sizeof(RmBvhNode)) + up(static_cast<size_t>(p.bvh_prim_count) * 4);
        if (p.cell_on) b += 2 * 16 + up(static_cast<size_t>(p.ct_words) * 4);
        else b += up(static_cast<size_t>(p.pq_cell_count) * 4) + up(static_cast<size_t>(p.pq_list_count) * 2 + 4);
    } else if (p.accel == 1) {
        b += up(static_cast<size_t>(p.oct_nodes) * sizeof(RmOctNode)) + up(static_cast<size_t>(p.oct_prim_count) * 4);
    }
    b += up(static_cast<size_t>(p.n_prims) * sizeof(RmSphere)) + up(static_cast<size_t>(p.n_prims) * 8);
    if (p.accel == 2 && p.step_box) b += up(static_cast<size_t>(3) * p.sb_stride * 4);
    return b + 16;
}

}

#ifndef RM_LENGTH_SQRT
RmV2Plan rm_v2_plan(const RmRenderParams &p_in) {
    RmRenderParams p = p_in;
    if (p.leaf_order) p.bvh_prim_count = 0;
    if (p.list_cap < 1) p.list_cap = 1;
    const bool want = p.accel == 2 && p.step_box != 0 && p.multi_step != 0 && p.sb_stride > 0;
    const bool want_cells = want && p.cell_on != 0 && p.ct_words > 0 && !p.general;
    auto pass = [&](bool with_table, bool with_cells = false, bool rel_allowed = true, int cap_most = 64) {
        RmRenderParams c = p;
        c.step_box = with_table ? 1 : 0;
        c.cell_on = with_cells ? 1 : 0;
        if (!rel_allowed) c.rel_boxes = 0;
        if (c.list_cap > cap_most) c.list_cap = cap_most;
        RmV2Plan r;
        r.step_box = c.step_box;
        r.cell_on = c.cell_on;
        r.cell_refused = 0;
        r.list_cap = c.list_cap;
        r.list_bytes = c.accel == 2 ? static_cast<size_t>(4) * c.list_cap * 128 : 0;
        r.scene_bytes = scene_lds_bytes(c);
        r.lds = c.nodes_in_lds != 0 && r.scene_bytes + r.list_bytes + 16 <= 64 * 1024;
        r.rel = false;
        r.tier = 0;
        r.refused = 0;
        const size_t rel_bytes = static_cast<size_t>(c.bvh_nodes) * 48;
        constexpr size_t kLdsPerCu = 160 * 1024, kGranule = 1280, kStatic = sizeof(WaveDiag) * 4;
        auto per_cu = [&](const RmV2Plan &v) {
            const size_t bytes = (v.lds ? v.scene_bytes : 0) + (v.rel ? rel_bytes + 16 : 0) + v.list_bytes + 16 + kStatic;
            const size_t n = kLdsPerCu / ((bytes + kGranule - 1) / kGranule * kGranule);
            return static_cast<int>(n < RM_V2_WAVES ? n : RM_V2_WAVES);
        };
        r.per_cu = per_cu(r);
        if (!(r.lds && c.accel == 2)) return r;
        auto budget_for = [&](size_t bytes) { return bytes / kGranule * kGranule - kStatic; };
        auto fits = [&](size_t extra, int cap, size_t budget) { return r.scene_bytes + extra + static_cast<size_t>(4) * cap * 128 + 16 <= budget; };
        auto trim = [&](size_t extra, size_t budget) {
            int cap = c.list_cap;
            while (cap > 12 && !fits(extra, cap, budget)) cap -= 1;
            return fits(extra, cap, budget) ? cap : 0;
        };
        size_t budgets[4];
        int nb = 0;
        if (c.lds_budget_kb > 0) budgets[nb++] = budget_for(static_cast<size_t>(c.lds_budget_kb) * 1024);
        else {
            budgets[nb++] = budget_for(kLdsPerCu / RM_V2_WAVES);
            budgets[nb++] = budget_for(kLdsPerCu / 5);
        }
        budgets[nb++] = budget_for(kLdsPerCu / 4);
        r.tier = nb;
        for (int b = 0; b < nb; ++b) {
            int cap = c.rel_boxes ? trim(rel_bytes + 16, budgets[b]) : 0;
            if (cap > 0) r.rel = true;
            else cap = trim(0, budgets[b]);
            if (cap > 0) {
                r.list_cap = cap;
                r.list_bytes = static_cast<size_t>(4) * cap * 128;
                r.tier = b;
                break;
            }
            r.rel = false;
        }
        r.per_cu = per_cu(r);
        return r;
    };
    RmV2Plan plain = pass(false);
    if (!want) return plain;
    RmV2Plan with_table = pass(true);
    if (with_table.lds == plain.lds && with_table.rel == plain.rel && with_table.tier <= plain.tier) {
        if (want_cells) {
            const RmV2Plan with_cells = pass(true, true, with_table.rel, with_table.list_cap);
            if (with_cells.lds && with_table.lds && with_cells.rel == with_table.rel && with_cells.tier <= with_table.tier &&
                with_cells.list_cap >= with_table.list_cap)
                return with_cells;
            with_table.cell_refused = 1;
        }
        return with_table;
    }
    plain.refused = 1;
    plain.cell_refused = want_cells ? 1 : 0;
    return plain;
}
#endif

#ifndef RM_LENGTH_SQRT
namespace {
__global__ __launch_bounds__(1024) void lpt_sort_kernel(const uint8_t *cost_prev, uint16_t *perm, int stride, int tiles_x, int tiles_y) {
    extern __shared__ unsigned char lpt_smem[];
    const int x = blockIdx.x;
    const int R = queue_rows(tiles_y, x);
    const int n = R * tiles_x;
    uint8_t *cost = lpt_smem;
    unsigned int *cnt = reinterpret_cast<unsigned int *>(lpt_smem + ((stride + 15) & ~15));
    __shared__ unsigned int sum_s, nz_s, base_s[4];
    if (threadIdx.x == 0) sum_s = nz_s = 0;
    __syncthreads();
    unsigned int sum = 0, nz = 0;
    for (int e = threadIdx.x; e < n; e += 1024) {
        const uint8_t c = cost_prev ? cost_prev[static_cast<size_t>(x) * stride + e] : 0;
        cost[e] = c;
        sum += c;
        nz += c != 0;
    }
    atomicAdd(&sum_s, sum);
    atomicAdd(&nz_s, nz);
    __syncthreads();
    const float mean = nz_s ? static_cast<float>(sum_s) / static_cast<float>(nz_s) : 1e9f;
    auto cls = [&](uint8_t c) { const float f = c; return f >= 4.f * mean ? 0 : (f >= 2.f * mean ? 1 : (f >= 1.25f * mean ? 2 : 3)); };
    const int chunk = (n + 1023) / 1024, e0 = threadIdx.x * chunk, e1 = min(n, e0 + chunk);
    unsigned int mine[4] = {0, 0, 0, 0};
    for (int e = e0; e < e1; ++e) mine[cls(cost[e])]++;
    for (int c = 0; c < 4; ++c) cnt[c * 1024 + threadIdx.x] = mine[c];
    __syncthreads();
    if (threadIdx.x < 4) {
        unsigned int run = 0;
        for (int t = 0; t < 1024; ++t) {
            const unsigned int v = cnt[threadIdx.x * 1024 + t];
            cnt[threadIdx.x * 1024 + t] = run;
            run += v;
        }
        base_s[threadIdx.x] = run;
    }
    __syncthreads();
    unsigned int start[4], acc = 0;
    for (int c = 0; c < 4; ++c) {
        start[c] = acc + cnt[c * 1024 + threadIdx.x];
        acc += base_s[c];
    }
    for (int e = e0; e < e1; ++e) {
        const int c = cls(cost[e]);
        perm[static_cast<size_t>(x) * stride + start[c]++] = static_cast<uint16_t>(e);
    }
}
}
hipError_t rm_launch_lpt_sort(const uint8_t *cost_prev, uint16_t *perm, int stride, int tiles_x, int tiles_y, hipStream_t stream) {
    const size_t shmem = static_cast<size_t>((stride + 15) & ~15) + 4 * 1024 * sizeof(unsigned int);
    hipLaunchKernelGGL(lpt_sort_kernel, dim3(RM_QUEUES), dim3(1024), shmem, stream, cost_prev, perm, stride, tiles_x, tiles_y);
    return hipGetLastError();
}
#endif

hipError_t RM_LEN_VARIANT(rm_launch_wave_distance)(const RmRenderParams &p, const float *points, int64_t n, double *dist, uint32_t *count, hipStream_t stream) {
    if (p.accel != 2 || p.general || p.bvh_nodes <= 0) return hipErrorInvalidValue;
    if (n <= 0) return hipSuccess;
    const dim3 grid(static_cast<unsigned>((n + 255) / 256)), block(256);
    if (p.uniform_radius) hipLaunchKernelGGL(wave_distance_kernel<true>, grid, block, 0, stream, p, points, n, dist, count);
    else hipLaunchKernelGGL(wave_distance_kernel<false>, grid, block, 0, stream, p, points, n, dist, count);
    return hipGetLastError();
}

hipError_t RM_LEN_VARIANT(rm_launch_render_v2)(const RmRenderParams &p_in, hipStream_t stream, const char **kernel_name, uint32_t *shape) {
    RmRenderParams p = p_in;
    const int rows = p.local_rows;
    if (kernel_name) *kernel_name = "";
    if (rows <= 0 || p.width <= 0) return hipSuccess;
    if (!p.tile_counters) return hipErrorInvalidValue;
    if (p.leaf_order) p.bvh_prim_count = 0;
    if (p.item_px != 64 && p.item_px != 128 && p.item_px != 256) p.item_px = 64;
    if (p.item_px < p.tile_w) p.item_px = p.tile_w;
    const int tw = p.tile_w;
    const bool wide = p.item_wide != 0 && tw < 64 && p.item_px > 64;
    const int iw = wide ? tw * (p.item_px / 64) : tw, th = wide ? 64 / tw : p.item_px / tw;
    const int tiles_x = (p.width + iw - 1) / iw;
    const int tiles_y = (rows + th - 1) / th;
    auto log2i = [](int v) { int l = 0; while ((1 << l) < v) ++l; return l; };
    if ((tw & (tw - 1)) != 0 || tiles_x <= 0 || static_cast<long long>(tiles_x) * (tiles_y + 8) >= (1ll << 31)) return hipErrorInvalidValue;
    p.tile_w_log2 = log2i(tw);
    p.tile_h_log2 = log2i(th);
    p.item_w_log2 = log2i(iw);
    p.sub_dx = wide ? tw : 0;
    p.sub_dy = wide ? 0 : 64 / tw;
    p.tiles_x = tiles_x;
    p.tiles_y = tiles_y;
    p.tiles_x_magic = tiles_x == 1 ? 0u : static_cast<uint32_t>((1ull << 32) / static_cast<unsigned long long>(tiles_x)) + 1u;
    const unsigned needed = static_cast<unsigned>((static_cast<long long>(tiles_x) * tiles_y + 3) / 4);
    unsigned resident = 0, blocks = 0;
    if (p.refill_threshold < 1) p.refill_threshold = 1;
    if (p.refill_threshold > 64) p.refill_threshold = 64;
    const RmV2Plan plan = rm_v2_plan(p);
    const bool lds = plan.lds, rel = plan.rel;
    p.list_cap = plan.list_cap;
    p.step_box = plan.step_box;
    p.cell_on = plan.cell_on;
    if (p.accel != 2 || !p.leaf_rects || !p.bvh_leaves || p.bvh_leaf_count <= 0 || p.bvh_leaf_count > RM_RECT_CULL_MAX_LEAVES ||
        p.width > 65536 || p.height > 65536)
        p.rect_cull = 0;
    const size_t list_bytes = plan.list_bytes, scene_bytes = plan.scene_bytes, rel_bytes = static_cast<size_t>(p.bvh_nodes) * 48;
    size_t shmem = (lds ? scene_bytes : 0) + (rel ? rel_bytes + 16 : 0) + list_bytes + 16;
    if (p.lds_fill && p.blocks_per_cu >= 2 && p.blocks_per_cu <= 8) {
        const size_t room = (160 * 1024 / static_cast<size_t>(p.blocks_per_cu)) / 1280 * 1280 - sizeof(WaveDiag) * 4;
        if (room > shmem && room <= 64 * 1024) shmem = room;
    }
    {
        const LdsLayout lay = lds_layout_host(p, p.accel, lds, rel && p.accel == 2);
        const uint32_t v[12] = {lay.nodes, lay.prims, lay.cells, lay.list, lay.oct, lay.oct_prims, lay.spheres, lay.radii, lay.rel, lay.end, lay.step, lay.ctab};
        for (int k = 0; k < 12; ++k) p.lds_off[k] = v[k];
        if (lay.end + list_bytes > shmem) return hipErrorInvalidValue;
    }
    const int cus = p.num_cus > 0 ? p.num_cus : 256;
    const int floor_per_cu = p.launch_per_cu > 0 ? p.launch_per_cu : p.blocks_per_cu;
    const int per_cu = rm_v2_overlap_per_cu(floor_per_cu, p.overlap_per_cu, static_cast<long long>(tiles_x) * tiles_y, cus);
    resident = static_cast<unsigned>(cus) * static_cast<unsigned>(per_cu > 0 ? per_cu : 4);
    blocks = needed < resident ? (needed ? needed : 1u) : resident;
    if (shape) {
        shape[0] = blocks;
        shape[1] = 256;
        shape[2] = static_cast<uint32_t>(shmem);
        shape[3] = p.step_box ? 1u : 0u;
        shape[4] = p.rect_cull ? 1u : 0u;
        shape[5] = p.cell_on ? 1u : 0u;
    }
    hipError_t e = hipSuccess;
    if (!p.diag_block) e = hipMemsetAsync(p.tile_counters, 0, RM_QUEUES * RM_QSTRIDE * sizeof(unsigned int), stream);
    if (e != hipSuccess) return e;
    p.lpt_perm = nullptr;
    if (p.lpt_perm_out) {
        const long long per_queue = static_cast<long long>(queue_rows_host(tiles_y, 0)) * tiles_x;
        if (per_queue <= p.lpt_stride && per_queue <= 32768) {
            e = rm_launch_lpt_sort(p.lpt_cost_prev, p.lpt_perm_out, p.lpt_stride, tiles_x, tiles_y, stream);
            if (e != hipSuccess) return e;
            p.lpt_perm = p.lpt_perm_out;
        } else {
            p.lpt_cost_out = nullptr;
        }
    } else {
        p.lpt_cost_out = nullptr;
    }
    const dim3 grid(blocks), block(256);
#define RM_V2X(A, L, U, R)                                                                                                   \
    {                                                                                                                        \
        const void *fn_ = p.rtc_ctx ? rm_rtc_v2_hook(p, A, L, U, R, RM_LEN_IS_SQRT) : nullptr;                               \
        if (fn_) {                                                                                                           \
            size_t bytes_ = sizeof p;                                                                                        \
            void *extra_[] = {HIP_LAUNCH_PARAM_BUFFER_POINTER, &p, HIP_LAUNCH_PARAM_BUFFER_SIZE, &bytes_, HIP_LAUNCH_PARAM_END}; \
            e = hipModuleLaunchKernel(reinterpret_cast<hipFunction_t>(const_cast<void *>(fn_)), grid.x, 1, 1, 256, 1, 1,     \
                                      static_cast<unsigned>(shmem), stream, nullptr, extra_);                               \
            if (e != hipSuccess) return e;                                                                                   \
            if (kernel_name) *kernel_name = "render_kernel_v2<" #A ", " #L ", " #U ", " #R ">" RM_LEN_TAG " [launch constants compiled in]"; \
        } else {                                                                                                             \
            hipLaunchKernelGGL((render_kernel_v2<A, L, U, R>), grid, block, shmem, stream, p);                               \
            if (kernel_name) *kernel_name = "render_kernel_v2<" #A ", " #L ", " #U ", " #R ">" RM_LEN_TAG;                   \
        }                                                                                                                    \
    }
#define RM_V2(A, L) RM_V2X(A, L, false, false)
    if (p.accel == 2) {
        if (lds && rel && p.uniform_radius) RM_V2X(2, true, true, true)
        else if (lds && rel) RM_V2X(2, true, false, true)
        else if (lds && p.uniform_radius) RM_V2X(2, true, true, false)
        else if (lds) RM_V2(2, true)
        else RM_V2(2, false)
    }
    else if (p.accel == 1) { if (lds) RM_V2(1, true) else RM_V2(1, false) }
    else { if (lds) RM_V2(0, true) else RM_V2(0, false) }
#undef RM_V2X
#undef RM_V2
    return hipGetLastError();
}
#endif
```

### cpu_raymarcher_amd/csrc/rm_types.h

```cpp
#pragma once
#ifndef __HIPCC_RTC__
#include <stdint.h>
#else
using __hip_internal::int8_t;
using __hip_internal::int16_t;
using __hip_internal::int32_t;
using __hip_internal::int64_t;
using __hip_internal::uint8_t;
using __hip_internal::uint16_t;
using __hip_internal::uint32_t;
using __hip_internal::uint64_t;
#endif

struct RmBvhNode {
    float lo[3];
    int32_t skip;
    float hi[3];
    int32_t leaf;
};

struct RmOctNode {
    float lo[3];
    int32_t first_child;
    float hi[3];
// ... 98 lines not shown
    int32_t item_px;
    int32_t local_rows;
    int32_t stripe_rows;
    int32_t n_parts, part;
    int32_t rel_boxes;
    const uint16_t *lpt_perm;
    uint8_t *lpt_cost_out;
    const uint8_t *lpt_cost_prev;
    uint16_t *lpt_perm_out;
    int32_t lpt_stride;
    int32_t launch_per_cu;
    int32_t v1_lists;
    int32_t v1_list_offset;
    uint32_t lds_off[12];
    int32_t prim_filter;
    int32_t n0_batch;
    const int32_t *stripe_ids;
    unsigned int *tile_counters;
    unsigned long long *stamps;
    const uint32_t *pq_cells;
    const uint16_t *pq_list;
    const uint16_t *bvh_leaves;
    int32_t bvh_leaf_count;
    int32_t v1_block;
    int32_t oct_lean;
    const uint32_t *nn_cells;
    const uint16_t *nn_list;
    int32_t nn_cell_count, nn_list_count, use_nn;
    int32_t tile_w_log2, tile_h_log2, tiles_x, tiles_y;
    int32_t item_wide, item_w_log2, sub_dx, sub_dy;
    const void *rtc_function;
    void *rtc_ctx;
    uint32_t tiles_x_magic;
    int32_t lds_budget_kb;
    int32_t leaf_order;
    int32_t nn_dim[3];
    float nn_inv[3];
    int32_t overlap_per_cu;
    const uint32_t *ext_cells;
    const uint16_t *ext_list;
    int32_t ext_dim[3];
    float ext_origin[3], ext_inv[3];
    int32_t use_ext;
    int32_t algorithm;
    int32_t general;
    int32_t uniform_radius;
    const RmPrim *prims;
    const RmInstr *prog;
    const int32_t *obj_ranges;
    int32_t prog_slots, prog_vals;
    double time;
    double overshoot;
    double step_size;
    const RmSphere *spheres;
    const double *radii;
    const RmBvhNode *bvh;
    const int32_t *bvh_prims;
    const RmOctNode *oct;
    const int32_t *oct_prims;
    const RmSphereRec *oct_recs;
    const int32_t *oct_lut;
    const RmOctFrameNode *oct_frame;
    const uint32_t *oct_sub_hdr;
    const uint8_t *oct_sub_list;
    uint8_t *depth;
    uint8_t *normal;
    uint16_t *sdf;
    uint16_t *iters;
    uint8_t *rgba;
    int32_t lds_fill;
    int32_t multi_step;
    RmDiagBlock *diag_block;
    RmDiagDevice *diag_out;
    const uint32_t *step_tab;
    float sb_origin[3], sb_inv[3];
    int32_t sb_bins, sb_stride;
    int32_t step_box;
    RmLeafRect *leaf_rects;
    int32_t rect_cull;
    const uint32_t *cell_tab;
    int32_t ct_dim[3];
    int32_t ct_rec_off, ct_list_off, ct_words;
    int32_t cell_on;
};
```

### cpu_raymarcher_amd/csrc/rm_v2_fields.h

```cpp
#pragma once

#define RM_V2_FIXED_SCALARS(X)                                                                                                  \
    X(width) X(height) X(accel) X(shader) X(tile_w) X(nodes_in_lds) X(filter) X(variant) X(list_cap) X(coop) X(use_grid)         \
    X(refill_threshold) X(hw_xcd) X(item_px) X(rel_boxes) X(lpt_stride) X(prim_filter) X(n0_batch) X(use_nn) X(tile_w_log2)     \
    X(tile_h_log2) X(tiles_x) X(item_wide) X(item_w_log2) X(sub_dx) X(sub_dy) X(tiles_x_magic) X(leaf_order) X(algorithm)       \
    X(general) X(uniform_radius) X(multi_step) X(use_ext) X(step_box) X(sb_bins) X(sb_stride) X(rect_cull) \
    X(ct_rec_off) X(ct_list_off) X(ct_words) X(cell_on)

#define RM_V2_FIXED_COUNTS(X)                                                                                                    \
    X(n_prims) X(bvh_nodes) X(oct_nodes) X(bvh_prim_count) X(oct_prim_count) X(pq_cell_count) X(pq_list_count) X(bvh_leaf_count) \
    X(nn_cell_count) X(nn_list_count)

#define RM_V2_FIXED_ARRAYS(X) \
    X(pq_dim, 3) X(lds_off, 12) X(nn_dim, 3) X(pq_origin, 3) X(pq_inv, 3) X(pq_cell, 3) X(nn_inv, 3) X(light, 3) X(light_d, 3) \
    X(ext_dim, 3) X(ext_origin, 3) X(ext_inv, 3) X(sb_origin, 3) X(sb_inv, 3) X(ct_dim, 3)
```

### include/rm_raymarch.h

```cpp
#ifndef RM_RAYMARCH_H
#define RM_RAYMARCH_H

#include <stddef.h>
#include <stdint.h>

#ifdef __cplusplus
extern "C" {
#endif

#define RM_API __attribute__((visibility("default")))

typedef struct rm_ctx rm_ctx;

typedef enum rm_status {
    RM_OK = 0,
    RM_E_INVALID = -1,
    RM_E_UNSUPPORTED = -2,
    RM_E_NO_DEVICE = -3,
    RM_E_HIP = -4,
    RM_E_NO_SCENE = -5,
    RM_E_NOMEM = -6
} rm_status;

typedef enum rm_accel { RM_ACCEL_NONE = 0, RM_ACCEL_OCTREE = 1, RM_ACCEL_BVH = 2 } rm_accel;
// ... 410 lines not shown
RM_API int rm_shade_ranged(rm_ctx *ctx, int32_t counter, int32_t width, int32_t rows, int32_t n_frames,
                           const uint16_t *values, const rm_frame_hist *hist, uint32_t lo, uint32_t hi,
                           uint8_t *rgba);

RM_API int rm_shade_lit_device(rm_ctx *ctx, int32_t width, int32_t rows, int32_t n_frames, const void *d_depth,
                               const void *d_normal, const void *d_lit, const void *d_ao, void *d_rgba, void *stream);
RM_API int rm_shade_lit(rm_ctx *ctx, int32_t width, int32_t rows, int32_t n_frames, const uint8_t *depth,
                        const uint8_t *normal, const float *lit, const float *ao, uint8_t *rgba);

typedef enum rm_field_map { RM_FIELD_MAP_DISTANCE = 0, RM_FIELD_MAP_COUNT = 1 } rm_field_map;
typedef struct rm_field_shade {
    int32_t  map, reserved;
    double   range;
    double   band;
    double   line;
    uint32_t lo, hi;
} rm_field_shade;
RM_API int rm_shade_field_device(rm_ctx *ctx, const rm_field_shade *shade, int64_t n, const void *d_values, void *d_rgba,
                                 void *stream);
RM_API int rm_shade_field(rm_ctx *ctx, const rm_field_shade *shade, int64_t n, const void *values, uint8_t *rgba);

RM_API int rm_render_stripes_device(rm_ctx *ctx, const rm_job *job, int32_t shader, int32_t stripe_rows,
                                    int32_t n_parts, int32_t part, void *d_depth, void *d_normal,
                                    void *d_sdf, void *d_iters, void *d_rgba, void *stream);
RM_API int rm_stripe_rows(int32_t y_start, int32_t y_end, int32_t stripe_rows, int32_t n_parts, int32_t part);

RM_API int rm_deal_stripes(int32_t rows, int32_t stripe_rows, int32_t n_parts, const int32_t *weights, int32_t *owner);

RM_API int rm_render_stripe_list_device(rm_ctx *ctx, const rm_job *job, int32_t shader, int32_t stripe_rows,
                                        const int32_t *stripe_ids, int32_t n_stripes, void *d_depth, void *d_normal,
                                        void *d_sdf, void *d_iters, void *d_rgba, void *stream);

RM_API int rm_assemble_frame_device(rm_ctx *ctx, const void *d_gathered, int64_t rank_stride, int64_t section_offset,
                                    int32_t row_bytes, int32_t height, int32_t stripe_rows, const int32_t *owner,
                                    int32_t n_stripes, int32_t world, void *d_frame, int64_t acc_offset, void *d_acc,
                                    void *stream);

RM_API int rm_shade(rm_ctx *ctx, int32_t shader, int32_t width, int32_t height,
                    const uint8_t *depth, const uint8_t *normal, const uint16_t *sdf,
                    const uint16_t *iters, uint8_t *rgba);
RM_API int rm_shade_device(rm_ctx *ctx, int32_t shader, int32_t width, int32_t height,
                           const void *d_depth, const void *d_normal, const void *d_sdf,
                           const void *d_iters, void *d_rgba, void *stream);

RM_API int rm_reduce_counters(rm_ctx *ctx, const uint16_t *sdf, const uint16_t *iters, int64_t n,
                              rm_diagnostics *out);
RM_API int rm_reduce_counters_device(rm_ctx *ctx, const void *d_sdf, const void *d_iters, int64_t n,
                                     rm_diagnostics *out, void *stream);

RM_API int rm_reduce_counters_enqueue(rm_ctx *ctx, const void *d_sdf, const void *d_iters, int64_t n,
                                      void *d_acc, void *stream);

RM_API int rm_render_attach_diagnostics(rm_ctx *ctx, void *d_acc);


RM_API int rm_partition_rows(int32_t height, int32_t n_workers, int32_t i, int32_t *y_start,
                             int32_t *y_end);


RM_API int rm_selftest_hypot(rm_ctx *ctx, const float *xyz, int64_t n, double *out);

RM_API int rm_selftest_jsmath(rm_ctx *ctx, int32_t fn, const double *a, const double *b, int64_t n, double *out);

RM_API int rm_selftest_hypot64(rm_ctx *ctx, const double *xyz, int64_t n, int32_t on_device, double *out);

RM_API int rm_selftest_fastdiv(rm_ctx *ctx, uint64_t seed, int64_t n, uint64_t *mismatches);

RM_API int rm_selftest_recip(rm_ctx *ctx, int mode, uint64_t *mismatches);

RM_API int rm_debug_read_stamps(rm_ctx *ctx, uint64_t *out8);

RM_API int rm_rtc_source(rm_ctx *ctx, char *out, int64_t cap, int64_t *needed);
RM_API int rm_rtc_compile_check(rm_ctx *ctx, int32_t accel, int32_t other, char *log, int64_t cap, double *seconds);
RM_API int rm_rtc_status(rm_ctx *ctx, int32_t *compiled, int32_t *failed, char *log, int64_t cap);

RM_API int rm_debug_read_counts(rm_ctx *ctx, uint64_t *out32);
RM_API int rm_debug_read_lpt_costs(rm_ctx *ctx, uint8_t *out, int64_t n);
RM_API int rm_debug_scene_table(rm_ctx *ctx, const char *name, int32_t from_device, void *out, int64_t cap, int64_t *bytes);
RM_API int rm_debug_launch_fill(rm_ctx *ctx, int32_t asked, int32_t *effective);
RM_API int rm_debug_last_launch(rm_ctx *ctx, uint32_t out[4]);
RM_API int rm_debug_overlap_fill(rm_ctx *ctx, int32_t asked, int64_t items, int32_t *effective);
RM_API int rm_debug_step_box(rm_ctx *ctx, int32_t out[6]);
RM_API int rm_debug_cell_tab(rm_ctx *ctx, int32_t out[12]);
RM_API int rm_debug_exact_tree(rm_ctx *ctx, int32_t out[4]);
RM_API int rm_debug_rect_cull(rm_ctx *ctx, const float *rot9, const float *origin3, int32_t width, int32_t height, int32_t out[5]);
RM_API int rm_debug_leaf_rects(rm_ctx *ctx, const float *rot9, const float *origin3, int32_t width, int32_t height,
                               uint16_t *rects, int32_t *nodes, int64_t cap, int64_t *n);
RM_API int rm_debug_read_wave_times(rm_ctx *ctx, uint64_t *out24576);
RM_API int rm_debug_read_batch_log(rm_ctx *ctx, uint32_t *out196608);

RM_API int rm_set_option(rm_ctx *ctx, const char *key, int64_t value);
RM_API int rm_get_option(const rm_ctx *ctx, const char *key, int64_t *value);

#ifdef __cplusplus
}
#endif
#endif
```

Baseline: 1795.

## Track runner-up sphere and third-best bound to extend cached multi-step marching

The uniform-radius BVH scan now keeps the three nearest sphere keys instead of two, and packs the second-nearest id plus a quantized lower bound for the third into the per-pixel aux word. When the cached step loop would otherwise stop because the second sphere might be closer, it evaluates that runner-up sphere exactly and keeps stepping if both it and the third bound stay farther. This is meant to avoid full BVH re-traversals for rays near two spheres. The cost is an extra sphere evaluation per check and more register pressure. It is enabled by default when the cell table is active.

```diff
diff --git a/cpu_raymarcher_amd/_native.py b/cpu_raymarcher_amd/_native.py
--- a/cpu_raymarcher_amd/_native.py
+++ b/cpu_raymarcher_amd/_native.py
@@ -313,6 +313,8 @@
     "rm_debug_overlap_fill": (C.c_int, [_VP, C.c_int32, C.c_int64, C.POINTER(C.c_int32)]),
     "rm_debug_step_box": (C.c_int, [_VP, C.POINTER(C.c_int32)]),
     "rm_debug_cell_tab": (C.c_int, [_VP, C.POINTER(C.c_int32)]),
+    "rm_debug_runner_up": (C.c_int, [_VP, C.POINTER(C.c_int32)]),
+    "rm_debug_scan_keys": (C.c_int, [_VP, C.c_int64, C.c_float, C.POINTER(C.c_uint32), C.POINTER(C.c_float), C.POINTER(C.c_float)]),
     "rm_debug_exact_tree": (C.c_int, [_VP, C.POINTER(C.c_int32)]),
     "rm_debug_rect_cull": (C.c_int, [_VP, _VP, _VP, C.c_int32, C.c_int32, C.POINTER(C.c_int32)]),
     "rm_debug_leaf_rects": (C.c_int, [_VP, _VP, _VP, C.c_int32, C.c_int32, _VP, _VP, C.c_int64, C.POINTER(C.c_int64)]),
diff --git a/cpu_raymarcher_amd/context.py b/cpu_raymarcher_amd/context.py
--- a/cpu_raymarcher_amd/context.py
+++ b/cpu_raymarcher_amd/context.py
@@ -234,6 +234,19 @@
         N.check(self._h, N.lib().rm_debug_cell_tab(self._h, out))
         return dict(last=bool(out[0]), planned=bool(out[1]), reason=out[2], list_cap=out[3], list_cap_without=out[4], table_bytes=out[5],
                     per_cu=out[6], scene_bytes=out[7], scene_bytes_without=out[8], cells=out[9], records=out[10], leaf_sets=out[11])
+
+    def runner_up(self):
+        out = (C.c_int32 * 4)()
+        N.check(self._h, N.lib().rm_debug_runner_up(self._h, out))
+        return dict(last=bool(out[0]), planned=bool(out[1]), reason=out[2])
+
+    @staticmethod
+    def scan_keys(keys, rf=0.5):
+        k = np.ascontiguousarray(keys, dtype=np.uint32).reshape(-1)
+        out = (C.c_uint32 * 3)()
+        lb3, carried = C.c_float(0.0), C.c_float(0.0)
+        N.check(None, N.lib().rm_debug_scan_keys(_ptr(k) if k.size else None, int(k.size), float(rf), out, C.byref(lb3), C.byref(carried)))
+        return [int(out[0]), int(out[1]), int(out[2])], lb3.value, carried.value
 
     def rect_cull(self, rot, origin, width, height):
         r = np.ascontiguousarray(rot, dtype=np.float32).reshape(9)
diff --git a/cpu_raymarcher_amd/csrc/rm_api.cpp b/cpu_raymarcher_amd/csrc/rm_api.cpp
--- a/cpu_raymarcher_amd/csrc/rm_api.cpp
+++ b/cpu_raymarcher_amd/csrc/rm_api.cpp
@@ -366,11 +366,12 @@
     int64_t opt_min_fill = 1;
     int64_t opt_overlap_fill = 1;
     int hw_queues = 4;
-    uint32_t last_v2_shape[6] = {0, 0, 0, 0, 0, 0};
+    uint32_t last_v2_shape[7] = {0, 0, 0, 0, 0, 0, 0};
     int64_t opt_item_wide = 0;
     int64_t opt_multi_step = 1;
     int64_t opt_step_box = 1;
     int64_t opt_cell_tab = 1;
+    int64_t opt_runner_up = 1;
     int64_t opt_lds_kb = 0;
     int64_t opt_refill = 64;
     int64_t opt_recs = 1;
@@ -1223,6 +1224,7 @@
     p.ct_words = static_cast<int32_t>(ctx->host.cell_tab.size());
     for (int k = 0; k < 3; ++k) p.ct_dim[k] = ctx->host.ct_dim[k];
     p.cell_on = (ctx->opt_cell_tab && p.step_box && !ctx->host.cell_tab.empty() && (ctx->dev.cell_tab || !ctx->has_device)) ? 1 : 0;
+    p.runner_up = (ctx->opt_runner_up && p.cell_on) ? 1 : 0;
     p.uniform_radius = 0;
     if (ctx->opt_uniform && !ctx->host.general && ctx->host.spheres.size() >= 2 &&
         ctx->host.spheres.size() <= 256) {
@@ -3794,6 +3796,42 @@
     return RM_OK;
 }
 
+int rm_debug_runner_up(rm_ctx *ctx, int32_t out[4]) {
+    if (!ctx || !out) return RM_E_INVALID;
+    for (int k = 0; k < 4; ++k) out[k] = 0;
+    out[0] = static_cast<int32_t>(ctx->last_v2_shape[6]);
+    if (!ctx->have_scene) return fail(ctx, RM_E_NO_SCENE, "no scene set");
+    rm_job job;
+    std::memset(&job, 0, sizeof job);
+    job.width = job.height = job.y_end = 64;
+    job.algorithm = RM_ALG_SPHERE_TRACER;
+    job.scene_preset_index = ctx->scene_is_uploaded ? RM_SCENE_UPLOADED : ctx->scene_preset;
+    job.acceleration_structure = ctx->host.accel;
+    job.overshoot_factor = job.step_size = std::nan("");
+    const double scene_time = ctx->time;
+    RmRenderParams p;
+    const int rc = fill_params(ctx, &job, p);
+    ctx->time = scene_time;
+    if (rc) return rc;
+    const RmV2Plan plan = rm_v2_plan(p);
+    const bool v2 = p.variant == 2 && p.algorithm == 0 && p.accel == 2;
+    out[1] = v2 && plan.runner_up ? 1 : 0;
+    out[2] = out[1] ? 0 : (!ctx->opt_runner_up ? 1 : (!(v2 && plan.cell_on) ? 2 : 3));
+    return RM_OK;
+}
+
+int rm_debug_scan_keys(const uint32_t *keys, int64_t n, float rf, uint32_t out3[3], float *lb3, float *lb3_carried) {
+    if (n < 0 || (n > 0 && !keys) || !out3 || !lb3 || !lb3_carried) return RM_E_INVALID;
+    RmScanKeys k = {0xFFFFFFFFu, 0xFFFFFFFFu, 0xFFFFFFFFu};
+    for (int64_t i = 0; i < n; ++i) rm_scan_keys_update(k, keys[i]);
+    out3[0] = k.best;
+    out3[1] = k.second;
+    out3[2] = k.third;
+    *lb3 = rm_scan_key_bound(k.third, rf);
+    *lb3_carried = rm_runner_up_unpack_bound(rm_runner_up_pack_bound(*lb3));
+    return RM_OK;
+}
+
 int rm_debug_exact_tree(rm_ctx *ctx, int32_t out[4]) {
     if (!ctx || !out) return RM_E_INVALID;
     for (int k = 0; k < 4; ++k) out[k] = 0;
@@ -3888,6 +3926,7 @@
     {"multi_step", &rm_ctx::opt_multi_step, kSwitch, {}, nullptr},
     {"step_box", &rm_ctx::opt_step_box, kSwitch, {}, nullptr},
     {"cell_tab", &rm_ctx::opt_cell_tab, kSwitch, {}, nullptr},
+    {"runner_up", &rm_ctx::opt_runner_up, kSwitch, {}, nullptr},
     {"item_wide", &rm_ctx::opt_item_wide, kSwitch, {}, nullptr},
     {"prune", &rm_ctx::opt_prune, kSwitch, {}, nullptr},
     {"rtc_spheres", &rm_ctx::opt_rtc_spheres, kRange, {0, 33}, "rtc_spheres must be 0..33"},
diff --git a/cpu_raymarcher_amd/csrc/rm_kernels.h b/cpu_raymarcher_amd/csrc/rm_kernels.h
--- a/cpu_raymarcher_amd/csrc/rm_kernels.h
+++ b/cpu_raymarcher_amd/csrc/rm_kernels.h
@@ -63,6 +63,34 @@
     return r;
 }
 
+struct RmScanKeys {
+    uint32_t best, second, third;
+};
+inline __host__ __device__ void rm_scan_keys_update(RmScanKeys &k, uint32_t key) {
+    const uint32_t lo = key < k.best ? key : k.best, hi = key < k.best ? k.best : key;
+    const uint32_t mid = hi < k.second ? k.second : hi;
+    k.best = lo;
+    k.second = hi < k.second ? hi : k.second;
+    k.third = mid < k.third ? mid : k.third;
+}
+inline __host__ __device__ uint32_t rm_scan_key(uint32_t s2_bits, uint32_t id) { return (s2_bits & 0xFFFFFF00u) | (id & 0xFFu); }
+inline __host__ __device__ float rm_scan_key_bound(uint32_t key, float rf) {
+    const float s2 = __builtin_bit_cast(float, key & 0xFFFFFF00u);
+#ifdef __HIP_DEVICE_COMPILE__
+    const float len = __builtin_amdgcn_sqrtf(s2);
+#else
+    const float len = __builtin_sqrtf(s2);
+#endif
+    const float lb = (len - rf) - (len + __builtin_fabsf(rf) + 1.0f) * 4e-6f;
+    return key != 0xFFFFFFFFu && s2 < __builtin_inff() ? lb : __builtin_inff();
+}
+inline __host__ __device__ uint32_t rm_runner_up_pack_bound(float lb3) {
+    const float mag = __builtin_fabsf(lb3);
+    const float low = lb3 - (mag < 3.0e38f ? mag : 3.0e38f) * 0.015625f;
+    return __builtin_bit_cast(uint32_t, low) & 0xFFFF0000u;
+}
+inline __host__ __device__ float rm_runner_up_unpack_bound(uint32_t word) { return __builtin_bit_cast(float, word & 0xFFFF0000u); }
+
 enum { RM_CMP_NONE = -1, RM_CMP_SDF = 0, RM_CMP_ITERS = 1, RM_CMP_DEPTH = 2, RM_CMP_NORMAL = 3, RM_CMP_SURFACE = 4 };
 struct RmCompareStats {
     unsigned long long pixels;
@@ -409,6 +437,7 @@
 struct RmV2Plan {
     bool lds, rel;
     int list_cap, step_box, tier, refused, cell_on, cell_refused;
+    int runner_up;
     int per_cu;
     size_t scene_bytes, list_bytes;
 };
diff --git a/cpu_raymarcher_amd/csrc/rm_render_v2.hip b/cpu_raymarcher_amd/csrc/rm_render_v2.hip
--- a/cpu_raymarcher_amd/csrc/rm_render_v2.hip
+++ b/cpu_raymarcher_amd/csrc/rm_render_v2.hip
@@ -18,7 +18,7 @@
             atomicAdd(&rm_cnt_s[(i) + 16], n_);                                                    \
         }                                                                                          \
     }
-__shared__ unsigned int rm_cnt_e[8];
+__shared__ unsigned int rm_cnt_e[16];
 #define RM_CNT_END(i)                                                                              \
     {                                                                                              \
         const unsigned int n_ = static_cast<unsigned int>(__popcll(__ballot(1)));                  \
@@ -292,17 +292,14 @@
 struct BestScan {
     int k1;
     float hi1, lb1, lb2;
-    uint32_t kbest, ksecond;
+    RmScanKeys keys;
 };
 template <bool UR>
 __device__ __forceinline__ void scan_sphere(BestScan &b, const RmSphere &s, int id, const Vec3f &p) {
     if (UR) {
         const float dx = p.x - s.cx, dy = p.y - s.cy, dz = p.z - s.cz;
         const float s2 = dx * dx + dy * dy + dz * dz;
-        const uint32_t key = (__float_as_uint(s2) & 0xFFFFFF00u) | static_cast<uint32_t>(id);
-        const uint32_t lo = min(key, b.kbest), hi = max(key, b.kbest);
-        b.kbest = lo;
-        b.ksecond = min(hi, b.ksecond);
+        rm_scan_keys_update(b.keys, rm_scan_key(__float_as_uint(s2), static_cast<uint32_t>(id)));
         return;
     }
     float err;
@@ -339,6 +336,7 @@
     const uint32_t *tab;
     const uint32_t *step;
     bool on;
+    bool ru;
 };
 __device__ __forceinline__ int cell_axis_index(const RmRenderParams &P, const uint32_t *step, int k, float x) {
     const uint32_t *axis = step + k * P.sb_stride;
@@ -368,7 +366,7 @@
     BestScan bs;
     bs.k1 = -1;
     bs.hi1 = bs.lb1 = bs.lb2 = __builtin_inff();
-    bs.kbest = bs.ksecond = 0xFFFFFFFFu;
+    bs.keys.best = bs.keys.second = bs.keys.third = 0xFFFFFFFFu;
     auto scan_leaf = [&](const RmBvhNode &node) {
         const int first = node.leaf >> 8, cnt = node.leaf & 0xFF;
         for (int k = 0; k < cnt; ++k) {
@@ -501,20 +499,26 @@
         }
     }
     bool redo = false;
-    if (UR && bs.kbest != 0xFFFFFFFFu) {
-        bs.k1 = static_cast<int>(bs.kbest & 0xFFu);
-        bs.lb2 = bs.ksecond == 0xFFFFFFFFu ? __builtin_inff() : __uint_as_float(bs.ksecond & 0xFFFFFF00u);
-    }
+    if (UR && bs.keys.best != 0xFFFFFFFFu) {
+        bs.k1 = static_cast<int>(bs.keys.best & 0xFFu);
+        bs.lb2 = bs.keys.second == 0xFFFFFFFFu ? __builtin_inff() : __uint_as_float(bs.keys.second & 0xFFFFFF00u);
+    }
+    float lb3 = __builtin_inff();
     if (bs.k1 >= 0) {
         RM_CNT(10)
         const RmSphere s1 = S.spheres[bs.k1];
         if (UR) scan_finish_uniform(bs, s1.rf);
+        if (UR && CT.ru) lb3 = rm_scan_key_bound(bs.keys.third, s1.rf);
         closest = sphere_sdf_fast(s1, S.radii[bs.k1], q);
         if (closest > RM_MAX_DIST) closest = RM_MAX_DIST;
         redo = bs.lb2 <= f32_upper_bound(closest);
     }
     {
         aux->k1 = bs.k1;
+        if (UR && CT.ru) {
+            const uint32_t k2 = bs.keys.second == 0xFFFFFFFFu ? bs.keys.best : bs.keys.second;
+            aux->k1 = static_cast<int>((bs.keys.best & 0xFFu) | ((k2 & 0xFFu) << 8) | rm_runner_up_pack_bound(lb3));
+        }
         aux->lb2 = bs.lb2;
         aux->found = (found & 0xFFFFu) | nleaf16;
         aux->rho = rho;
@@ -1022,7 +1026,7 @@
 #endif
 #ifdef RM_COUNTS
     if (threadIdx.x < 32) rm_cnt_s[threadIdx.x] = 0;
-    if (threadIdx.x < 8) rm_cnt_e[threadIdx.x] = 0;
+    if (threadIdx.x < 16) rm_cnt_e[threadIdx.x] = 0;
     __syncthreads();
 #endif
     for (;;) {
@@ -1279,11 +1283,13 @@
         aux.rho = 0.f;
         aux.rho_cell = 0.f;
         const bool cell_on = ACCEL == 2 && CB.cell_on != 0;
+        const bool ru = UR && cell_on && CB.runner_up != 0;
         if (ACCEL == 2) {
             CellTabView CT;
             CT.tab = LDS ? reinterpret_cast<const uint32_t *>(smem + CB.lds_off[11]) : CB.cell_tab;
             CT.step = LDS ? reinterpret_cast<const uint32_t *>(smem + CB.lds_off[10]) : CB.step_tab;
             CT.on = cell_on;
+            CT.ru = ru;
 #ifdef RM_STAMPS
             unsigned long long fbc = 0;
             dist = bvh_distance_wave<UR>(CB, SB, need, q, evaluated, lane_b, coop, filter, use_grid, &fbc, &aux, CT);
@@ -1331,8 +1337,9 @@
                 if (go) {
                     const RmRenderParams CM = cold_params();
                     const SceneView SM = scene_view<ACCEL, LDS, REL>(CM, smem);
-                    const RmSphere s1 = SM.spheres[aux.k1];
-                    const double r1 = SM.radii[aux.k1];
+                    const int k1 = ru ? aux.k1 & 0xFF : aux.k1;
+                    const RmSphere s1 = SM.spheres[k1];
+                    const double r1 = SM.radii[k1];
                     const bool step_box = CM.step_box != 0;
                     float b_lo[3], b_hi[3];
                     if (step_box && CM.cell_on) {
@@ -1414,9 +1421,20 @@
                         const float ex = p2.x - q.x, ey = p2.y - q.y, ez = p2.z - q.z;
                         const float dd = __builtin_amdgcn_sqrtf(ex * ex + ey * ey + ez * ez) * 1.00001f + 1e-7f;
                         const double e = sphere_sdf_fast(s1, r1, p2);
-                        if (!(aux.lb2 - dd > f32_upper_bound(e))) {
-                            RM_CNT_END(3)
-                            break;
+                        const float e_up = f32_upper_bound(e);
+                        if (!(aux.lb2 - dd > e_up)) {
+                            bool farther = false;
+                            if (ru) {
+                                float err2;
+                                const float a2 = sphere_sdf_estimate(SM.spheres[(aux.k1 >> 8) & 0xFF], p2, err2);
+                                farther = __builtin_fminf(a2 - err2, rm_runner_up_unpack_bound(static_cast<uint32_t>(aux.k1)) - dd) > e_up;
+                            }
+                            if (!farther) {
+                                RM_CNT_END(3)
+                                if (ru) RM_CNT_END(9)
+                                break;
+                            }
+                            RM_CNT_END(8)
                         }
                         RM_CNT(15)
                         st += 1 << ST_TRIP_SHIFT;
@@ -1449,8 +1467,9 @@
             }
             if (fuse && stable) {
                 const SceneView SN = scene_view<ACCEL, LDS, REL>(cold_params(), smem);
-                const RmSphere s1 = SN.spheres[aux.k1];
-                const double r1 = SN.radii[aux.k1];
+                const int k1 = ru ? aux.k1 & 0xFF : aux.k1;
+                const RmSphere s1 = SN.spheres[k1];
+                const double r1 = SN.radii[k1];
                 Vec3f qx = q, qy = q, qz = q;
                 qx.x = to_f32(static_cast<double>(q.x) - 0.01);
                 qy.y = to_f32(static_cast<double>(q.y) - 0.01);
@@ -1491,7 +1510,7 @@
 #ifdef RM_COUNTS
     __syncthreads();
     if (threadIdx.x < 32 && P.stamps) atomicAdd(&P.stamps[8 + threadIdx.x], static_cast<unsigned long long>(rm_cnt_s[threadIdx.x]));
-    if (threadIdx.x < 8 && P.stamps) atomicAdd(&P.stamps[40 + threadIdx.x], static_cast<unsigned long long>(rm_cnt_e[threadIdx.x]));
+    if (threadIdx.x < 16 && P.stamps) atomicAdd(&P.stamps[40 + threadIdx.x], static_cast<unsigned long long>(rm_cnt_e[threadIdx.x]));
 #endif
 }
 
@@ -1517,7 +1536,7 @@
     const SceneView S = scene_view<2, false, false>(P, nullptr);
     uint32_t c = 0;
     NormalAux aux;
-    const CellTabView CT = {P.cell_tab, P.step_tab, P.cell_on != 0};
+    const CellTabView CT = {P.cell_tab, P.step_tab, P.cell_on != 0, false};
     const double d = bvh_distance_wave<UR>(P, S, need, q, c, static_cast<int>(threadIdx.x & 63), P.coop != 0, P.filter != 0, P.use_grid != 0, nullptr, &aux, CT);
     if (need) {
         dist[i] = d;
@@ -1559,6 +1578,7 @@
         r.step_box = c.step_box;
         r.cell_on = c.cell_on;
         r.cell_refused = 0;
+        r.runner_up = c.cell_on && c.runner_up != 0 && c.uniform_radius != 0 ? 1 : 0;
         r.list_cap = c.list_cap;
         r.list_bytes = c.accel == 2 ? static_cast<size_t>(4) * c.list_cap * 128 : 0;
         r.scene_bytes = scene_lds_bytes(c);
@@ -1724,6 +1744,7 @@
     p.list_cap = plan.list_cap;
     p.step_box = plan.step_box;
     p.cell_on = plan.cell_on;
+    p.runner_up = plan.runner_up;
     if (p.accel != 2 || !p.leaf_rects || !p.bvh_leaves || p.bvh_leaf_count <= 0 || p.bvh_leaf_count > RM_RECT_CULL_MAX_LEAVES ||
         p.width > 65536 || p.height > 65536)
         p.rect_cull = 0;
@@ -1751,6 +1772,7 @@
         shape[3] = p.step_box ? 1u : 0u;
         shape[4] = p.rect_cull ? 1u : 0u;
         shape[5] = p.cell_on ? 1u : 0u;
+        shape[6] = p.runner_up ? 1u : 0u;
     }
     hipError_t e = hipSuccess;
     if (!p.diag_block) e = hipMemsetAsync(p.tile_counters, 0, RM_QUEUES * RM_QSTRIDE * sizeof(unsigned int), stream);
diff --git a/cpu_raymarcher_amd/csrc/rm_types.h b/cpu_raymarcher_amd/csrc/rm_types.h
--- a/cpu_raymarcher_amd/csrc/rm_types.h
+++ b/cpu_raymarcher_amd/csrc/rm_types.h
@@ -204,4 +204,5 @@
     int32_t ct_dim[3];
     int32_t ct_rec_off, ct_list_off, ct_words;
     int32_t cell_on;
-};
+    int32_t runner_up;
+};
diff --git a/cpu_raymarcher_amd/csrc/rm_v2_fields.h b/cpu_raymarcher_amd/csrc/rm_v2_fields.h
--- a/cpu_raymarcher_amd/csrc/rm_v2_fields.h
+++ b/cpu_raymarcher_amd/csrc/rm_v2_fields.h
@@ -5,7 +5,7 @@
     X(refill_threshold) X(hw_xcd) X(item_px) X(rel_boxes) X(lpt_stride) X(prim_filter) X(n0_batch) X(use_nn) X(tile_w_log2)     \
     X(tile_h_log2) X(tiles_x) X(item_wide) X(item_w_log2) X(sub_dx) X(sub_dy) X(tiles_x_magic) X(leaf_order) X(algorithm)       \
     X(general) X(uniform_radius) X(multi_step) X(use_ext) X(step_box) X(sb_bins) X(sb_stride) X(rect_cull) \
-    X(ct_rec_off) X(ct_list_off) X(ct_words) X(cell_on)
+    X(ct_rec_off) X(ct_list_off) X(ct_words) X(cell_on) X(runner_up)
 
 #define RM_V2_FIXED_COUNTS(X)                                                                                                    \
     X(n_prims) X(bvh_nodes) X(oct_nodes) X(bvh_prim_count) X(oct_prim_count) X(pq_cell_count) X(pq_list_count) X(bvh_leaf_count) \
diff --git a/include/rm_raymarch.h b/include/rm_raymarch.h
--- a/include/rm_raymarch.h
+++ b/include/rm_raymarch.h
@@ -516,6 +516,8 @@
 RM_API int rm_debug_overlap_fill(rm_ctx *ctx, int32_t asked, int64_t items, int32_t *effective);
 RM_API int rm_debug_step_box(rm_ctx *ctx, int32_t out[6]);
 RM_API int rm_debug_cell_tab(rm_ctx *ctx, int32_t out[12]);
+RM_API int rm_debug_runner_up(rm_ctx *ctx, int32_t out[4]);
+RM_API int rm_debug_scan_keys(const uint32_t *keys, int64_t n, float rf, uint32_t out3[3], float *lb3, float *lb3_carried);
 RM_API int rm_debug_exact_tree(rm_ctx *ctx, int32_t out[4]);
 RM_API int rm_debug_rect_cull(rm_ctx *ctx, const float *rot9, const float *origin3, int32_t width, int32_t height, int32_t out[5]);
 RM_API int rm_debug_leaf_rects(rm_ctx *ctx, const float *rot9, const float *origin3, int32_t width, int32_t height,
```

Result: faster. 1851, median of 6 (+3.1%).
